# ritobanrc/firework

Measured on AMD Instinct MI355X. Metric: Mrays/s, cornell_box 512x512 @1024spp (scene resident in HBM; whole frame incl. tile gather), higher is better.
Workload: dtype f32; 1 GPU; C2_cornell_box 512x512 @1024spp; use_bvh=False, tiles=16x16, dealt diagonally over ranks, collective=none, rng=counter (pcg4d) keyed by (seed,pixel,sample,dimension), seed=0

## Files before the change

### firework_amd/csrc/fw_device.h

```cpp
#pragma once
#include <hip/hip_runtime.h>
#include <stdint.h>

#ifndef FW_AB
#define FW_AB 0
#endif

namespace fw {

constexpr int OBJ_Q = 6;

enum : uint32_t {
    OF_ROTATED = 1u << 0,
    OF_FLIP = 1u << 1,
    OF_RECT_FLIP = 1u << 2,
    OF_MESH_NORMALS = 1u << 3,
    OF_MESH_ATTR = 1u << 4,
    OF_CULL0 = 1u << 6,
    OF_GATE = 1u << 5,
};

constexpr uint32_t REF_LEAF = 0x80000000u, REF_DONE = 0xffffffffu;
constexpr int WIDE_NONE = 0, WIDE_F32 = 1, WIDE_Q8 = 2;
constexpr uint32_t WIDE_F32_DW = 28, WIDE_Q8_DW = 12;
// ... 226 lines not shown
    X(SHADE_GX_NEE_00_PL, "k_shade_gx_nee<0,0,pl>", -1) \
    X(SHADE_GX_NEE_01_PL, "k_shade_gx_nee<0,1,pl>", -1) \
    X(SHADE_GX_NEE_00_LS, "k_shade_gx_nee<0,0,ls>", -1) \
    X(SHADE_GX_NEE_01_LS, "k_shade_gx_nee<0,1,ls>", -1) \
    X(SHADE_GX_NEE_00_DL, "k_shade_gx_nee<0,0,dl>", -1) \
    X(SHADE_GX_NEE_01_DL, "k_shade_gx_nee<0,1,dl>", -1) \
    X(SHADE_GX_NEE_10_PL_ENV, "k_shade_gx_nee<1,0,pl_env>", -1) \
    X(SHADE_GX_NEE_10_ENV, "k_shade_gx_nee<1,0,env>", -1) \
    X(SHADE_GX_NEE_10_PL, "k_shade_gx_nee<1,0,pl>", -1) \
    X(SHADE_GX_NEE_11_PL, "k_shade_gx_nee<1,1,pl>", -1) \
    X(SHADE_GX_NEE_10_LS, "k_shade_gx_nee<1,0,ls>", -1) \
    X(SHADE_GX_NEE_11_LS, "k_shade_gx_nee<1,1,ls>", -1) \
    X(SHADE_GX_NEE_10_DL, "k_shade_gx_nee<1,0,dl>", -1) \
    X(SHADE_GX_NEE_11_DL, "k_shade_gx_nee<1,1,dl>", -1) \
    X(SHADE_GX_NEE_20_PL_ENV, "k_shade_gx_nee<2,0,pl_env>", -1) \
    X(SHADE_GX_NEE_20_ENV, "k_shade_gx_nee<2,0,env>", -1) \
    X(SHADE_GX_NEE_20_PL, "k_shade_gx_nee<2,0,pl>", -1) \
    X(SHADE_GX_NEE_21_PL, "k_shade_gx_nee<2,1,pl>", -1) \
    X(SHADE_GX_NEE_20_LS, "k_shade_gx_nee<2,0,ls>", -1) \
    X(SHADE_GX_NEE_21_LS, "k_shade_gx_nee<2,1,ls>", -1) \
    X(SHADE_GX_NEE_20_DL, "k_shade_gx_nee<2,0,dl>", -1) \
    X(SHADE_GX_NEE_21_DL, "k_shade_gx_nee<2,1,dl>", -1) \
    X(SHADOW_RESOLVE, "k_shadow_resolve", -1) \
    X(SHADOW_RESOLVE_ENV, "k_shadow_resolve_env", -1) \
    X(SHADOW_RESOLVE_PL, "k_shadow_resolve_pl", -1) \
    X(SHADOW_RESOLVE_DL, "k_shadow_resolve_dl", -1) \
    X(SHADOW_RESOLVE_GX, "k_shadow_resolve_gx", -1)
#if FW_AB
#define FW_KERNEL_IDS_AB(X) \
    X(EXTEND_BVH, "k_extend_bvh", -1) \
    X(SHADE_020, "k_shade<0,2,no chain>", -1) \
    X(SHADE_120, "k_shade<1,2,no chain>", -1) \
    X(SHADE_220, "k_shade<2,2,no chain>", -1) \
    X(BOUNCE_00, "k_bounce<false,false>", -1) \
    X(BOUNCE_01, "k_bounce<false,true>", -1) \
    X(BOUNCE_10, "k_bounce<true,false>", -1) \
    X(BOUNCE_11, "k_bounce<true,true>", -1)
#else
#define FW_KERNEL_IDS_AB(X)
#endif
#define FW_KERNEL_IDS(X) FW_KERNEL_IDS_PRODUCT(X) FW_KERNEL_IDS_AB(X)
enum KernelId : uint32_t {
#define FW_KID_ENUM(id, name, fam) KID_##id,
    FW_KERNEL_IDS(FW_KID_ENUM)
#undef FW_KID_ENUM
    KID_COUNT
};
constexpr uint32_t KID_N_WALK = 26;
extern const char *const KERNEL_NAMES[KID_COUNT];
extern const signed char KERNEL_FAMILY[KID_COUNT];
struct KernelLog {
    uint64_t bits[(KID_COUNT + 63) / 64];
    uint8_t waves[KID_COUNT];
    void clear() { *this = KernelLog{}; }
    void add(KernelId id) { bits[id >> 6] |= 1ull << (id & 63u); }
    void add(KernelId id, uint32_t w) { add(id); waves[id] |= (uint8_t)(w == 16u ? 1u : w == 12u ? 2u : 4u); }
    void merge(const KernelLog &o) { for (size_t i = 0; i < sizeof bits / sizeof bits[0]; i++) bits[i] |= o.bits[i]; for (uint32_t i = 0; i < KID_COUNT; i++) waves[i] |= o.waves[i]; }
    bool has(uint32_t id) const { return ((bits[id >> 6] >> (id & 63u)) & 1u) != 0; }
};

struct LaunchCfg {
    hipStream_t stream;
    DQueue q;
    int blocks_other;
    int tlas_depth, blas_depth;
    uint32_t n_mat, n_tex;
    bool lds_tables;
    bool has_mesh;
    bool simple_but_meshes;
    bool simple_set;
    int n_cus;
    uint32_t blas_pair_nodes, tlas_pair_nodes, max_tris, n_tris;
    bool no_lds_tris;
    uint32_t n_defer;
    bool lds_trees;
    int shade_mode;
    int exact_form;
    uint32_t ref_tlas_nodes, ref_blas_nodes, ref_tlas_depth, ref_blas_depth;
    int wblas_fmt, wtlas_fmt;
    uint32_t wblas_nodes, wtlas_nodes, wblas_depth, wtlas_depth;
    uint32_t debug_wide_levels;
    bool gx;
    KernelLog *log;
    bool tlas_refill;
};
constexpr size_t LDS_TREE_LIMIT = 160 * 1024;
constexpr size_t LDS_TABLE_LIMIT = 16 * 1024;

void launch_raygen(const LaunchCfg &, const DCamera &, const DFrame &, DPaths out, float4 *sample_rad, uint32_t n_paths);
void launch_raygen_views(const LaunchCfg &, const DCamera *cams, uint32_t n_view, const DFrame &, DPaths out, float4 *sample_rad, uint32_t n_paths);
void launch_resolve_views(const LaunchCfg &, const DFrame &, uint32_t n_view, const float4 *accum, uint32_t total_spp, float gamma,
                          uint8_t *rgb8, float *gamma_rgb, float *linear_rgb);
void launch_view_ids(hipStream_t stream, const uint32_t *src, uint32_t n_view, uint32_t n, uint32_t *out);
void launch_raygen_rays(const LaunchCfg &, const float *rays, bool per_sample, uint32_t *err, const DFrame &, DPaths out, uint32_t n_paths);
void launch_ray_keys(hipStream_t stream, uint32_t base, uint32_t n, uint32_t *out);
void launch_extend(const LaunchCfg &, const DScene &, const DFrame &, DPaths in, float2 *hits, int segment, bool use_bvh, DPark park);
void launch_extend_exact(const LaunchCfg &, const DScene &, const DFrame &, const DPaths &in, float2 *hits, int segment, bool use_bvh);
void launch_shade(const LaunchCfg &, const DScene &, const DFrame &, DPaths in, DPaths out, const float2 *hits,
                  float4 *sample_rad, int segment);
void launch_shade_nee(const LaunchCfg &, const DScene &, const DFrame &, DPaths in, DPaths out, const float2 *hits,
                      float4 *sample_rad, int segment, const DShadow &, const DEnvDist *ed, const DEmitters *em, const DDeltaLights *dl = nullptr);
void launch_shadow_resolve(const LaunchCfg &, const DScene &, const DShadow &, const float2 *hits, int segment, bool env, bool pl, bool dl = false,
                           float4 *sample_rad = nullptr);
int build_env_dist(hipStream_t stream, const DEnv &env, float *cdf_m, float *cdf_c, float *dens, float *p_out, double *scratch, double *total);
void launch_env_sample_test(hipStream_t stream, const DEnv &env, const DEnvDist &ed, uint32_t n, uint32_t seed32, float *out);
void launch_emitter_weights(hipStream_t stream, const DScene &sc, const uint4 *ent, uint32_t n, float *w);
void launch_emitter_sample_test(hipStream_t stream, const DScene &sc, const DEmitters &em, float x, float y, float z, uint32_t n, uint32_t seed32, float *out);
void launch_ggx_test(hipStream_t stream, uint32_t n, const float *in, float *out);
void launch_bounce(const LaunchCfg &, const DScene &, const DFrame &, DPaths in, DPaths out, float4 *sample_rad, int segment,
                   bool use_bvh);
void launch_queue_totals(const LaunchCfg &, uint32_t *totals, const uint32_t *ptotal);
void launch_trace_load(const LaunchCfg &, const DFrame &, const float *rays, DPaths out, uint32_t n, uint32_t key0, uint32_t *ids, uint32_t *slot_of);
void launch_trace_store(const LaunchCfg &, const DScene &, const DFrame &, const DPaths &in, const float2 *hits, const uint32_t *slot_of, uint32_t n,
                        float4 *out);
void launch_camera_rays(hipStream_t stream, int n_cus, const DCamera &, const DFrame &, uint32_t n, float *out);
void launch_aov_accumulate(hipStream_t stream, int n_cus, const DScene &, const DFrame &, const DPaths &in, const float2 *hits, const uint32_t *slot_of,
                           uint32_t n, uint32_t first, float4 *sum);
void launch_aov_finish(hipStream_t stream, int n_cus, uint32_t n, uint32_t spp, float4 *aov);
void launch_hit_surface(hipStream_t stream, int n_cus, const DScene &, uint32_t n_mat, const float *rays, const float4 *hits, uint32_t n, float4 *surface);
void launch_denoise(hipStream_t stream, int n_cus, uint32_t W, uint32_t H, uint32_t L, const float *color, const float4 *aov, const float4 *moments,
                    float4 *guide, float4 *ev0, float4 *ev1, float gamma, uint8_t *rgb8, float *gamma_rgb, float *linear_rgb);
void launch_scatter_tiles(hipStream_t stream, const uint32_t *ids, uint32_t n, const uint8_t *in8, const float *ing, const float *inl,
                          uint8_t *out8, float *outg, float *outl);
void launch_tile_order(hipStream_t stream, uint32_t width, uint32_t height, uint32_t *ids);
void launch_upload(hipStream_t stream, const void *pinned_src, void *dst, size_t bytes);
#if FW_AB
uint32_t take_error_word();
#endif
void preload_kernels();
void launch_count_deposits(const LaunchCfg &, const uint32_t *dep_bits, uint32_t *total);
void launch_selftest_arith(hipStream_t stream, uint32_t n, uint32_t seed, int mode, unsigned long long *out);
void launch_selftest_libm(hipStream_t stream, int fn, uint32_t n, const float *x, const float *y, float *out);
void launch_accumulate(const LaunchCfg &, const DFrame &, const float4 *sample_rad, float4 *accum);
void launch_resolve(const LaunchCfg &, const DFrame &, const float4 *accum, uint32_t total_spp, float gamma,
                    uint8_t *rgb8, float *gamma_rgb, float *linear_rgb);
constexpr uint32_t ADAPTIVE_MAX_BLOCKS = 1024;
void launch_accumulate_adaptive(const LaunchCfg &, const DFrame &, const float4 *sample_rad, float4 *accum, float4 *moments);
uint32_t adaptive_select_blocks(uint32_t n);
void launch_adaptive_select(hipStream_t stream, const uint32_t *ids, uint32_t n, const float4 *accum, float4 *moments, uint32_t n_samples, bool may_continue,
                            float tol, unsigned long long *mask, uint32_t *block_counts, uint32_t *out_ids, uint32_t *count);
void launch_resolve_adaptive(hipStream_t stream, int n_cus, uint32_t n, const float4 *accum, const float4 *moments, float gamma,
                             uint8_t *rgb8, float *gamma_rgb, float *linear_rgb);

constexpr int BLOCK = 256;

}
```

### firework_amd/csrc/fw_kernels.hip

```cpp
#include "../../include/firework_hip.h"
#include "fw_device.h"
#include "fw_libm.h"
#include "fw_defer_pretest.h"
#include <atomic>
#include <type_traits>

namespace fw {

struct V3 { float x, y, z; };
__device__ __forceinline__ V3 mk(float x, float y, float z) { return V3{x, y, z}; }
__device__ __forceinline__ V3 operator+(V3 a, V3 b) { return {a.x + b.x, a.y + b.y, a.z + b.z}; }
__device__ __forceinline__ V3 operator-(V3 a, V3 b) { return {a.x - b.x, a.y - b.y, a.z - b.z}; }
__device__ __forceinline__ V3 operator-(V3 a) { return {-a.x, -a.y, -a.z}; }
__device__ __forceinline__ V3 operator*(V3 a, V3 b) { return {a.x * b.x, a.y * b.y, a.z * b.z}; }
__device__ __forceinline__ V3 operator*(float s, V3 a) { return {s * a.x, s * a.y, s * a.z}; }
__device__ __forceinline__ V3 operator*(V3 a, float s) { return {a.x * s, a.y * s, a.z * s}; }
__device__ __forceinline__ float dot(V3 a, V3 b) { return fmaf(a.x, b.x, fmaf(a.y, b.y, a.z * b.z)); }
__device__ __forceinline__ V3 cross(V3 a, V3 b) {
    return {fmaf(a.y, b.z, -a.z * b.y), fmaf(a.z, b.x, -a.x * b.z), fmaf(a.x, b.y, -a.y * b.x)};
}
__device__ __forceinline__ float mag_sq(V3 a) { return dot(a, a); }
__device__ __forceinline__ float comp(V3 a, int i) { return i == 0 ? a.x : (i == 1 ? a.y : a.z); }
__device__ __forceinline__ V3 ld3(const float *p) { return {p[0], p[1], p[2]}; }

// ... 325 lines not shown
        const uint32_t slot = w * q.cap + chunk * 64u + lane;
        bool fl = false; V3 o = mk(0, 0, 0), d = o;
        if (i < n_paths) {
            const Ray r = camera_ray(cam, f, key_of_linear(f, i));
            o = r.o; d = r.d;
            if (f.pinhole0) qst(&out.ray_a[slot], make_float4(d.x, d.y, d.z, 0.f));
            else {
                qst(&out.ray_a[slot], make_float4(o.x, o.y, o.z, d.x));
                qst(&out.ray_b[slot], make_float2(d.y, d.z));
            }
            fl = f.ex.mode && needs_exact(f.ex, o.x, o.y, o.z, d.x, d.y, d.z);
        }
        if (f.ex.mode) flag_exact(f.ex, fl, slot, 0);
        produced += min(64u, n_paths - id0);
    }
    if (lane == 0) q.wcount[w] = produced;
}

__global__ __launch_bounds__(WB) void k_raygen_views(const DCamera *__restrict__ cams, uint32_t n_view, DFrame f, DPaths out,
                                                     float4 *__restrict__ sample_rad, DQueue q, uint32_t n_paths) {
    const uint32_t w = wave_index(), lane = threadIdx.x & 63u;
    if (w >= q.n_waves) return;
    uint32_t produced = 0;
    for (uint32_t chunk = 0;; chunk++) {
        uint32_t id0 = chunk * (q.n_waves * 64u) + w * 64u;
        if (id0 >= n_paths) break;
        uint32_t i = id0 + lane;
        const uint32_t slot = w * q.cap + chunk * 64u + lane;
        bool fl = false; V3 o = mk(0, 0, 0), d = o;
        if (i < n_paths) {
            uint32_t s_local = (uint32_t)((float)i * f.inv_n_pixels);
            int32_t p_local = (int32_t)(i - s_local * f.n_pixels);
            if (p_local < 0) p_local += (int32_t)f.n_pixels; else if ((uint32_t)p_local >= f.n_pixels) p_local -= (int32_t)f.n_pixels;
            const DCamera cam = cams[(uint32_t)p_local / n_view];
            const Ray r = camera_ray(cam, f, key_of_linear(f, i));
            o = r.o; d = r.d;
            if (f.pinhole0) qst(&out.ray_a[slot], make_float4(d.x, d.y, d.z, 0.f));
            else {
                qst(&out.ray_a[slot], make_float4(o.x, o.y, o.z, d.x));
                qst(&out.ray_b[slot], make_float2(d.y, d.z));
            }
            fl = f.ex.mode && needs_exact(f.ex, o.x, o.y, o.z, d.x, d.y, d.z);
        }
        if (f.ex.mode) flag_exact(f.ex, fl, slot, 0);
        produced += min(64u, n_paths - id0);
    }
    if (lane == 0) q.wcount[w] = produced;
}

struct Obj { float4 q0, q1, q2, q3, q4; uint32_t kf, material, aux0, aux1; };

__device__ __forceinline__ Obj load_obj(const float4 *__restrict__ objs, uint32_t j) {
    const float4 *p = objs + (size_t)j * OBJ_Q;
    float4 r0 = p[0], r3 = p[3], r4 = p[4], r5 = p[5];
    Obj o;
    o.q0 = make_float4(r3.x, r3.y, r3.z, r0.x); o.q1 = make_float4(r4.x, r4.y, r4.z, r0.y); o.q2 = make_float4(r5.x, r5.y, r5.z, r0.z);
    o.q3 = p[1]; o.q4 = p[2];
    o.kf = __float_as_uint(r0.w); o.material = __float_as_uint(r3.w);
    o.aux0 = __float_as_uint(r4.w); o.aux1 = __float_as_uint(r5.w);
    return o;
}
__device__ __forceinline__ Obj load_obj_for_hit(const float4 *__restrict__ objs, uint32_t j) {
    const float4 *p = objs + (size_t)j * OBJ_Q;
    float4 r0 = p[0];
    Obj o;
    o.kf = __float_as_uint(r0.w); o.material = 0; o.aux0 = 0; o.aux1 = 0;
    o.q0 = make_float4(1.f, 0.f, 0.f, r0.x); o.q1 = make_float4(0.f, 1.f, 0.f, r0.y); o.q2 = make_float4(0.f, 0.f, 1.f, r0.z);
    o.q3 = p[1]; o.q4 = make_float4(0.f, 0.f, 0.f, 0.f);
    const uint32_t kind = o.kf & 0xffu, flags = (o.kf >> 8) & 0xffffu, inner = o.kf >> 24;
    if (kind == 1u || kind == 2u || kind == 3u || kind == 4u || kind == 6u) o.q4 = p[2];
    const bool mesh = kind == 5u || (kind == 6u && inner == 5u);
    if ((flags & OF_ROTATED) || mesh) {
        float4 r3 = p[3], r4 = p[4], r5 = p[5];
        o.q0 = make_float4(r3.x, r3.y, r3.z, r0.x); o.q1 = make_float4(r4.x, r4.y, r4.z, r0.y); o.q2 = make_float4(r5.x, r5.y, r5.z, r0.z);
        o.aux0 = __float_as_uint(r4.w); o.aux1 = __float_as_uint(r5.w);
    }
    return o;
}
__device__ __forceinline__ uint32_t obj_kind(const Obj &o) { return o.kf & 0xffu; }
__device__ __forceinline__ uint32_t obj_flags(const Obj &o) { return (o.kf >> 8) & 0xffffu; }
__device__ __forceinline__ uint32_t obj_inner(const Obj &o) { return o.kf >> 24; }

__device__ __forceinline__ V3 rot_inv(const Obj &o, V3 v) {
    return {o.q0.x * v.x + o.q1.x * v.y + o.q2.x * v.z,
            o.q0.y * v.x + o.q1.y * v.y + o.q2.y * v.z,
            o.q0.z * v.x + o.q1.z * v.y + o.q2.z * v.z};
}
__device__ __forceinline__ V3 rot_fwd(const Obj &o, V3 v) {
    return {o.q0.x * v.x + o.q0.y * v.y + o.q0.z * v.z,
            o.q1.x * v.x + o.q1.y * v.y + o.q1.z * v.z,
            o.q2.x * v.x + o.q2.y * v.y + o.q2.z * v.z};
}
__device__ __forceinline__ Ray to_object_space(const Obj &o, const Ray &r) {
    V3 pos = mk(o.q0.w, o.q1.w, o.q2.w);
    if (obj_flags(o) & OF_ROTATED) return Ray{rot_inv(o, r.o - pos), rot_inv(o, r.d)};
    return Ray{r.o - pos, r.d};
}

__device__ __forceinline__ bool hit_sphere(float radius, const Ray &r, float tmin, float tmax, float &t_out) {
    float a = dot(r.d, r.d);
    float b = 2.f * dot(r.o, r.d);
    float c = dot(r.o, r.o) - radius * radius;
    float disc = b * b - 4.f * a * c;
    if (disc < 0.f) return false;
    float t1, t2; bool two;
    Rcp two_a = make_rcp(2.f * a);
// ... 867 lines not shown
        const float4 ra = ra_n; const float2 rb = rb_n;
        if (j + 64u < n) { ra_n = qld(&in.ray_a[i + 64u]); rb_n = load_ray_b(in, i + 64u, f, segment); }
        const bool active = j < n;
        bool deferred = false, have = false; uint32_t deferred_obj = 0, best_obj = MISS, best_prim = 0; float best_t = TMAX;
        Ray r{mk(0, 0, 0), mk(0, 0, 1)};
        if (active) {
            r = make_ray(ra, rb, f, segment);
            RngKey key{0, 0, 0};
            if (sc.has_medium) key = key_of(f, __float_as_uint(load_home(in, i, f, segment)));
            const V3 inv = mk(fdiv(1.f, r.d.x), fdiv(1.f, r.d.y), fdiv(1.f, r.d.z));
            const bool soft = sc.has_mesh && soft_ray(f.ex, r.d, sc.soft_shear);
            const uint32_t n_obj = skip_ray(f.ex, r) ? 0u : sc.n_objects;
            for (uint32_t k = 0; k < n_obj; k++) {
                const float4 lo = sc.obj_leaf[2 * (size_t)k], hi = sc.obj_leaf[2 * (size_t)k + 1];
                float entry;
                if (!hit_aabb_entry(lo, hi, r.o, inv, relaxed(inv), box_tmin(TMIN, soft), TMAX, entry) || entry > (soft ? NO_CULL : cull_bound(have ? best_t : TMAX))) continue;
                Obj o = load_obj(sc.obj, k);
                if (PARK && obj_kind(o) == 5u) {
                    if (obj_gate_ok(sc, k, r.o, inv)) { deferred = true; deferred_obj |= 1u << k; }
                    continue;
                }
                float t; uint32_t prim;
                if (PLAIN ? hit_object<false, 0, false, SIMPLE>(sc, o, k, r, TMIN, TMAX, nullptr, key, segment, t, prim) : hit_object(sc, o, k, r, TMIN, TMAX, blas_stack, key, segment, t, prim)) {
                    if ((!have || t < best_t || (t == best_t && sc.obj_rank[k] > sc.obj_rank[best_obj])) && obj_gate_ok(sc, k, r.o, inv)) { have = true; best_t = t; best_obj = k; best_prim = prim; }
                }
            }
            if (!deferred) qst(&hits[i], pack_hit(best_t, best_obj, best_prim, sc.prim_bits));
        }
        if (PARK) {
            const unsigned long long pmask = __ballot(deferred);
            if (pmask) {
                const uint32_t prank = __builtin_amdgcn_mbcnt_hi((uint32_t)(pmask >> 32), __builtin_amdgcn_mbcnt_lo((uint32_t)pmask, 0u));
                if (deferred) {
                    const uint32_t e = w * park_stride + park_n + prank;
                    qst(&park_a[e], make_float4(r.o.x, r.o.y, r.o.z, r.d.x));
                    qst(&park_b[e], make_float2(r.d.y, r.d.z));
                    qst(&park_m[e], make_float4(__uint_as_float(i), __uint_as_float(PARK_MASK | deferred_obj), best_t, pack_hit(best_t, best_obj, best_prim, sc.prim_bits).y));
                }
                park_n += (uint32_t)__popcll(pmask);
            }
        }
    }
    if (PARK && lane == 0) park_count[w] = park_n;
}

constexpr uint32_t DEFER_FIELDS = 9;
extern __shared__ uint32_t lds_defer[];
template <bool SIMPLE>
__global__ __launch_bounds__(WB) __attribute__((amdgpu_waves_per_eu(FW_DEFER_WAVES, 8)))
void k_extend_linear_defer(DScene sc, DFrame f, DPaths in, float2 *__restrict__ hits, DQueue q, int segment, uint32_t n_def) {
    const uint32_t w = wave_index(), lane = threadIdx.x & 63u;
    if (w >= q.n_waves) return;
    const uint32_t n = q.wcount[(size_t)segment * q.n_waves + w], base = w * q.cap;
    const float TMIN = 0.001f, TMAX = 2e9f;
    const uint32_t n_first = sc.n_objects - n_def;
    uint32_t *const L0 = lds_defer, *const L1 = lds_defer + DEFER_FIELDS * 64u;
    uint32_t cnt0 = 0, cnt1 = 0;
    const RngKey nokey{0, 0, 0};
    auto write_final = [&](uint32_t slot, float t, uint32_t code) {
        if (f.hit4) reinterpret_cast<uint32_t *>(hits)[slot] = code; else qst(&hits[slot], make_float2(t, __uint_as_float(code)));
    };
    auto put = [&](uint32_t *L, uint32_t e, uint32_t sb, float t, uint32_t code, const Ray &r) {
        L[e] = sb; L[64u + e] = __float_as_uint(t); L[128u + e] = code;
        L[192u + e] = __float_as_uint(r.o.x); L[256u + e] = __float_as_uint(r.o.y); L[320u + e] = __float_as_uint(r.o.z);
        L[384u + e] = __float_as_uint(r.d.x); L[448u + e] = __float_as_uint(r.d.y); L[512u + e] = __float_as_uint(r.d.z);
    };
    auto get = [&](const uint32_t *L, uint32_t e, uint32_t &sb, float &t, uint32_t &code, Ray &r) {
        sb = L[e]; t = __uint_as_float(L[64u + e]); code = L[128u + e];
        r.o = mk(__uint_as_float(L[192u + e]), __uint_as_float(L[256u + e]), __uint_as_float(L[320u + e]));
        r.d = mk(__uint_as_float(L[384u + e]), __uint_as_float(L[448u + e]), __uint_as_float(L[512u + e]));
    };
    auto test = [&](uint32_t d, const Ray &r, float &t, uint32_t &code) {
        const uint32_t k = n_first + d;
        const Obj o = load_obj(sc.obj, k);
        float tt; uint32_t prim;
        if (hit_rect3d(o.q3, o.q4, to_object_space(o, r), TMIN, t, tt, prim)) { t = tt; code = (k << sc.prim_bits) | prim; }
    };
    auto append = [&](uint32_t *L, uint32_t &cnt, bool want, uint32_t sb, float t, uint32_t code, const Ray &r) {
        const unsigned long long m = __ballot(want);
        if (!m) return;
        const uint32_t rank = __builtin_amdgcn_mbcnt_hi((uint32_t)(m >> 32), __builtin_amdgcn_mbcnt_lo((uint32_t)m, 0u));
        if (want) put(L, cnt + rank, sb, t, code, r);
        cnt += (uint32_t)__popcll(m);
    };
    auto make_room = [&](uint32_t need0, uint32_t need1) {
        const bool r0 = cnt0 != 0u && cnt0 + need0 > 64u;
        const uint32_t pass_on = r0 ? (uint32_t)__popcll(__ballot(lane < cnt0 && (L0[lane] >> 31) != 0u)) : 0u;
#pragma nounroll
        for (int phase = 0; phase < 2; phase++) {
            const bool r1 = cnt1 != 0u && (phase == 0 ? cnt1 + pass_on > 64u : cnt1 + need1 > 64u);
            if (r1) {
                uint32_t sb = 0, code = MISS; float t = TMAX; Ray r{mk(0, 0, 0), mk(0, 0, 1)};
                if (lane < cnt1) { get(L1, lane, sb, t, code, r); test(1, r, t, code); write_final(sb, t, code); }
                cnt1 = 0;
            }
            if (phase == 0 && r0) {
                uint32_t sb = 0, code = MISS; float t = TMAX; Ray r{mk(0, 0, 0), mk(0, 0, 1)};
                const bool on = lane < cnt0;
                if (on) { get(L0, lane, sb, t, code, r); test(0, r, t, code); }
                cnt0 = 0;
                const bool more = on && (sb >> 31) != 0u;
                const uint32_t slot = sb & 0x7fffffffu;
                if (on && !more) write_final(slot, t, code);
                append(L1, cnt1, more, slot, t, code, r);
            }
        }
    };
    float4 ra_n = make_float4(0, 0, 0, 0); float2 rb_n = make_float2(0, 0);
    if (lane < n) { ra_n = qld(&in.ray_a[base + lane]); rb_n = load_ray_b(in, base + lane, f, segment); }
    for (uint32_t c0 = 0; c0 < n; c0 += 64u) {
        const uint32_t j = c0 + lane, i = base + j;
        const float4 ra = ra_n; const float2 rb = rb_n;
        if (j + 64u < n) { ra_n = qld(&in.ray_a[i + 64u]); rb_n = load_ray_b(in, i + 64u, f, segment); }
        const bool active = j < n;
        float best_t = TMAX; uint32_t best_obj = MISS, best_prim = 0;
        bool may0 = false, may1 = false;
        const Ray r = make_ray(ra, rb, f, segment);
        if (active) {
            const float4 *op = sc.obj;
            const Rcp rcx = make_rcp(r.d.x), rcy = make_rcp(r.d.y), rcz = make_rcp(r.d.z);
            for (uint32_t k = 0; k < n_first; k++, op += OBJ_Q) {
                const Obj o = load_obj(op, 0);
                float t; uint32_t prim = 0; bool h;
                const uint32_t kind = obj_kind(o);
                if (kind >= 1u && kind <= 3u && !(obj_flags(o) & OF_ROTATED) && o.q4.y == 0.f) {
                    const Ray ro{r.o - mk(o.q0.w, o.q1.w, o.q2.w), r.d};
                    if (kind == 1u) h = hit_rect_rcp<0>(o.q3.x, o.q3.y, o.q3.z, o.q3.w, o.q4.x, ro, rcz, TMIN, best_t, t);
                    else if (kind == 2u) h = hit_rect_rcp<1>(o.q3.x, o.q3.y, o.q3.z, o.q3.w, o.q4.x, ro, rcy, TMIN, best_t, t);
                    else h = hit_rect_rcp<2>(o.q3.x, o.q3.y, o.q3.z, o.q3.w, o.q4.x, ro, rcx, TMIN, best_t, t);
                } else h = hit_object<false, 0, false, SIMPLE>(sc, o, k, r, TMIN, best_t, nullptr, nokey, segment, t, prim);
                if (h) { best_t = t; best_obj = k; best_prim = prim; }
            }
            const fwpt::RayTerms rt = fwpt::ray_terms(r.o.x, r.o.y, r.o.z, rcx.r, rcy.r, rcz.r);
            const float4 *const cb = sc.obj_cull + 2 * ((size_t)sc.n_objects + n_first);
            may0 = fwpt::pretest_fma(rt, cb[0].x, cb[0].y, cb[0].z, cb[1].x, cb[1].y, cb[1].z, best_t);
            if (n_def > 1u) may1 = fwpt::pretest_fma(rt, cb[2].x, cb[2].y, cb[2].z, cb[3].x, cb[3].y, cb[3].z, best_t);
        }
        const uint32_t code = best_obj == MISS ? MISS : ((best_obj << sc.prim_bits) | best_prim);
        const bool c1 = may1 && !may0;
        make_room((uint32_t)__popcll(__ballot(may0)), (uint32_t)__popcll(__ballot(c1)));
        if (active && !may0 && !may1) write_final(i, best_t, code);
        append(L0, cnt0, may0, i | (may1 ? 0x80000000u : 0u), best_t, code, r);
        append(L1, cnt1, c1, i, best_t, code, r);
    }
    make_room(65u, 65u);
}

__global__ __launch_bounds__(WB) __attribute__((amdgpu_waves_per_eu(7, 8)))
void k_extend_linear(DScene sc, DFrame f, DPaths in, float2 *__restrict__ hits, DQueue q, int segment, int tlas_levels, int stack_levels) {
    extend_body<false, false, false>(sc, f, in, hits, q, segment, tlas_levels, stack_levels, DPark{});
}
__global__ __launch_bounds__(WB) __attribute__((amdgpu_waves_per_eu(7, 8)))
void k_extend_linear_nomesh(DScene sc, DFrame f, DPaths in, float2 *__restrict__ hits, DQueue q, int segment, int tlas_levels, int stack_levels) {
    extend_body<false, false, false, false>(sc, f, in, hits, q, segment, tlas_levels, stack_levels, DPark{});
}
__global__ __launch_bounds__(WB) __attribute__((amdgpu_waves_per_eu(7, 8)))
void k_extend_linear_plain(DScene sc, DFrame f, DPaths in, float2 *__restrict__ hits, DQueue q, int segment, int tlas_levels, int stack_levels) {
    extend_body<false, false, false, false, false>(sc, f, in, hits, q, segment, tlas_levels, stack_levels, DPark{});
}
template <bool MEDIUM>
__global__ __launch_bounds__(WB) __attribute__((amdgpu_waves_per_eu(7, 8)))
void k_extend_linear_simple(DScene sc, DFrame f, DPaths in, float2 *__restrict__ hits, DQueue q, int segment, int tlas_levels, int stack_levels) {
    extend_body<false, false, false, false, MEDIUM, true>(sc, f, in, hits, q, segment, tlas_levels, stack_levels, DPark{});
}
#if FW_AB
__global__ __launch_bounds__(WB) __attribute__((amdgpu_waves_per_eu(5, 8)))
void k_extend_bvh(DScene sc, DFrame f, DPaths in, float2 *__restrict__ hits, DQueue q, int segment, int tlas_levels, int stack_levels) {
    extend_body<true, false, false>(sc, f, in, hits, q, segment, tlas_levels, stack_levels, DPark{});
}
#endif
__global__ __launch_bounds__(WB) __attribute__((amdgpu_waves_per_eu(FW_TLAS_WAVES, 8)))
void k_extend_tlas(DScene sc, DFrame f, DPaths in, float2 *__restrict__ hits, DQueue q, int segment, int tlas_levels, int stack_levels) {
    extend_body<true, true, false>(sc, f, in, hits, q, segment, tlas_levels, stack_levels, DPark{});
}
__global__ __launch_bounds__(WB) __attribute__((amdgpu_waves_per_eu(FW_TLAS_WAVES, 8)))
void k_extend_tlas_park(DScene sc, DFrame f, DPaths in, float2 *__restrict__ hits, DQueue q, int segment, int tlas_levels, int stack_levels, DPark park) {
    extend_body<true, true, true>(sc, f, in, hits, q, segment, tlas_levels, stack_levels, park);
}

__global__ __launch_bounds__(WB) __attribute__((amdgpu_waves_per_eu(FW_BLAS_WAVES, 8)))
void k_blas(DScene sc, DPark park, float2 *__restrict__ hits, DQueue q) {
    const uint32_t w = wave_index(), lane = threadIdx.x & 63u;
    if (w >= q.n_waves) return;
    TS_BEGIN();
    const uint32_t n = park.pcount[w];
    if (lane == 0 && n) park.ptotal[w] += n;
    const uint32_t base = w * park.stride;
    const float TMIN = 0.001f, TMAX = 2e9f;
    float4 ca = make_float4(0, 0, 0, 0), na = ca, cm = ca, nm = ca; float2 cb = make_float2(0, 0), nb = cb;
    auto fetch = [&](uint32_t j, float4 &a, float2 &b, float4 &m) {
        if (j < n) { a = qld(&park.ray_a[base + j]); b = qld(&park.ray_b[base + j]); m = qld(&park.meta[base + j]); }
    };
    fetch(lane, ca, cb, cm); fetch(64u + lane, na, nb, nm);
    uint32_t cur_base = 0, q_next = 0;
    bool act = false, have = false;
    uint32_t slot = 0, obj = 0, tri_base = 0, bcode = MISS, mtri = 0, cur = REF_DONE;
    float bt = TMAX, mbest = TMAX;
    V3 ro = mk(0, 0, 0), inv = ro;
// ... 1454 lines not shown
                    }
                }
            }
            if (CHAIN) nchain = chain | (o.material << (f.chain_bits * (uint32_t)segment));
            else {
                nbeta = beta * atten;
                if (f.atten && alive) f.atten[(size_t)segment * f.atten_stride + path_id] = make_float4(atten.x, atten.y, atten.z, 0.f);
            }
            PH_ADD(5);
        }
    }
#ifdef FW_ABL_NO_DEPOSIT
    if (false) {
#else
    if (!alive && !(f.skip_zero_deposits && rad.x == 0.f && rad.y == 0.f && rad.z == 0.f)) {
#endif
        PH_T0;
        const float len = (float)(segment + 1);
        if (LS) { const float4 e = sh->nee[path_id]; rad = rad + mk(e.x, e.y, e.z); }
        if (FW_NT_RAD) st_nt(&sample_rad[path_id], make_float4(rad.x, rad.y, rad.z, len));
        else sample_rad[path_id] = make_float4(rad.x, rad.y, rad.z, len);
        if (f.skip_zero_deposits) {
            const uint32_t b = f.dep_pixel_major ? dep_bit_of(f, path_id) : path_id;
            atomicOr(&f.dep_bits[b >> 5], 1u << (b & 31u));
        }
        PH_ADD(6);
    }
    return alive;
}

extern __shared__ float4 lds_tables[];

template <int LDS_TAB, int MODE, bool CHAIN>
#ifndef FW_SHADE_WAVES
#define FW_SHADE_WAVES 5
#endif
#ifndef FW_SHADE_PIPE
#define FW_SHADE_PIPE 0
#endif
#ifndef FW_SHADE_STATIC_STORES
#define FW_SHADE_STATIC_STORES FW_SHADE_PIPE
#endif
__attribute__((amdgpu_waves_per_eu(FW_SHADE_WAVES, 8)))
__global__ __launch_bounds__(WB) void k_shade(DScene sc, DFrame f, DPaths in, DPaths out, const float2 *__restrict__ hits,
                                                 float4 *__restrict__ sample_rad, DQueue q, int segment,
                                                 uint32_t n_mat, uint32_t n_tex) {
    const uint32_t w = wave_index(), lane = threadIdx.x & 63u;
    __shared__ uint16_t shade_list[128];
#include "fw_shade_tables.inc"
    if (w >= q.n_waves) return;
    const uint32_t n = q.wcount[(size_t)segment * q.n_waves + w];
    const uint32_t base = w * q.cap;
    uint32_t out_n = 0;
    uint32_t list_n = 0;
    PH_DECL;
    auto compact = [&](bool alive, const Ray &nr, V3 nbeta, uint32_t nchain, uint32_t path_id, uint32_t c0 = 0xffffffffu) {
        const unsigned long long mask = __ballot(alive);
        const uint32_t rank = __builtin_amdgcn_mbcnt_hi((uint32_t)(mask >> 32), __builtin_amdgcn_mbcnt_lo((uint32_t)mask, 0u));
#if FW_SHADE_STATIC_STORES
        if (c0 != 0xffffffffu) {
#if FW_SHADE_STATIC_STORES == 2
            const uint32_t dst = base + (alive ? out_n + rank : q.cap - 1u);
#else
            const uint32_t dst = base + (alive ? out_n + rank : min(c0 + 64u + lane, q.cap - 1u));
#endif
            qst(&out.ray_a[dst], make_float4(nr.o.x, nr.o.y, nr.o.z, nr.d.x));
            qst(&out.ray_b[dst], make_float2(nr.d.y, nr.d.z));
            if (CHAIN) qst(&reinterpret_cast<float2 *>(out.state)[dst], make_float2(__uint_as_float(nchain), __uint_as_float(path_id)));
            else qst(&out.state[dst], make_float4(nbeta.x, nbeta.y, nbeta.z, __uint_as_float(path_id)));
        } else
#endif
        if (alive) {
            const uint32_t dst = base + out_n + rank;
            qst(&out.ray_a[dst], make_float4(nr.o.x, nr.o.y, nr.o.z, nr.d.x));
            qst(&out.ray_b[dst], make_float2(nr.d.y, nr.d.z));
            if (CHAIN) qst(&reinterpret_cast<float2 *>(out.state)[dst], make_float2(__uint_as_float(nchain), __uint_as_float(path_id)));
            else qst(&out.state[dst], make_float4(nbeta.x, nbeta.y, nbeta.z, __uint_as_float(path_id)));
        }
        if (f.ex.mode)
            flag_exact(f.ex, alive && needs_exact(f.ex, nr.o.x, nr.o.y, nr.o.z, nr.d.x, nr.d.y, nr.d.z), base + out_n + rank, segment + 1);
        out_n += (uint32_t)__popcll(mask);
    };
    auto load_st = [&](uint32_t idx) { return CHAIN ? load_state_chain(in, idx, segment) : load_state(in, idx, segment); };
    auto load_hit = [&](uint32_t idx) { return f.hit4 ? make_float2(0.f, __uint_as_float(reinterpret_cast<const uint32_t *>(hits)[idx])) : qld(&hits[idx]); };
    auto run_list = [&](uint32_t take) {
        bool alive = false;
        Ray nr{mk(0, 0, 0), mk(0, 0, 0)}; V3 nbeta = mk(0, 0, 0); uint32_t path_id = 0, nchain = 0;
        if (lane < take) {
            const uint32_t i = base + shade_list[list_n - take + lane];
            const float4 ra = qld(&in.ray_a[i]), st = load_st(i); const float2 rb = load_ray_b(in, i, f, segment), hr = load_hit(i);
            path_id = __float_as_uint(st.w);
            alive = shade_path<false, CHAIN>(sc, f, objp, matp, texp, make_ray(ra, rb, f, segment), mk(st.x, st.y, st.z), __float_as_uint(st.x), path_id, hr.x, __float_as_uint(hr.y), segment, sample_rad, nr, nbeta, nchain PH_PASS);
        }
        list_n -= take;
        compact(alive, nr, nbeta, nchain, path_id);
    };
    float4 ra_n = make_float4(0, 0, 0, 0), st_n = ra_n; float2 rb_n = make_float2(0, 0), hr_n = rb_n;
#if FW_SHADE_PIPE
    auto prefetch = [&](uint32_t jn) {
        const uint32_t in_ = base + jn;
        ra_n = qld(&in.ray_a[in_]);
        rb_n = qld(&in.ray_b[short_rays(f, segment) ? base : in_]);
        if (CHAIN) { const float2 v = qld(&reinterpret_cast<const float2 *>(in.state)[segment == 0 ? base : in_]); st_n = make_float4(v.x, 0.f, 0.f, v.y); }
        else st_n = qld(&in.state[segment == 0 ? base : in_]);
        hr_n = load_hit(in_);
    };
    auto fix_implicit = [&](float4 &st_, float2 &rb_, uint32_t slot) {
        if (segment == 0) st_ = CHAIN ? make_float4(0.f, 0.f, 0.f, __uint_as_float(slot)) : make_float4(1.f, 1.f, 1.f, __uint_as_float(slot));
        if (short_rays(f, segment)) rb_ = make_float2(0.f, 0.f);
    };
    if (n) {
        prefetch(min(lane, n - 1u));
        const uint32_t d0 = base + lane;
        qst(&out.ray_a[d0], make_float4(0.f, 0.f, 0.f, 0.f));
        qst(&out.ray_b[d0], make_float2(0.f, 0.f));
        if (CHAIN) qst(&reinterpret_cast<float2 *>(out.state)[d0], make_float2(0.f, 0.f)); else qst(&out.state[d0], make_float4(0.f, 0.f, 0.f, 0.f));
    }
#else
    if (lane < n) { ra_n = qld(&in.ray_a[base + lane]); rb_n = load_ray_b(in, base + lane, f, segment); st_n = load_st(base + lane); hr_n = load_hit(base + lane); }
#endif
    for (uint32_t c0 = 0; c0 < n; c0 += 64u) {
        const uint32_t j = c0 + lane;
        const uint32_t i = base + j;
        float4 ra = ra_n, st = st_n; float2 rb = rb_n, hr = hr_n;
#if FW_SHADE_PIPE
        fix_implicit(st, rb, i);
        const RngKey key_ = key_of(f, __float_as_uint(st.w));
        prefetch(min(j + 64u, n - 1u));
        const RngKey *pre_key = &key_;
#else
        if (j + 64u < n) { ra_n = qld(&in.ray_a[i + 64u]); rb_n = load_ray_b(in, i + 64u, f, segment); st_n = load_st(i + 64u); hr_n = load_hit(i + 64u); }
        const RngKey *pre_key = nullptr;
#endif
        bool alive = false, later = false;
        Ray nr{mk(0, 0, 0), mk(0, 0, 0)}; V3 nbeta = mk(0, 0, 0); uint32_t path_id = 0, nchain = 0;
        if (j < n) {
            PH_T0;
            Ray r = make_ray(ra, rb, f, segment);
            V3 beta = mk(st.x, st.y, st.z);
            path_id = __float_as_uint(st.w);
            const uint32_t hit_code = __float_as_uint(hr.y);
#ifdef FW_ABL_SHADE_COPY
            alive = hit_code != MISS && segment < 10; nr = r; nbeta = beta; nchain = __float_as_uint(st.x) + (pre_key ? pre_key->pixel & 1u : 0u);
#else
            if (MODE == 2 && expensive_shading(sc, objp, matp, hit_code)) later = true;
            else alive = shade_path<MODE != 0, CHAIN>(sc, f, objp, matp, texp, r, beta, __float_as_uint(st.x), path_id, hr.x, hit_code, segment, sample_rad, nr, nbeta, nchain PH_PASS, pre_key);
#endif
            PH_ADD(0);
        }
        { PH_T0; compact(alive, nr, nbeta, nchain, path_id, c0); PH_ADD(7); }
        if (MODE == 2) {
            const unsigned long long lm = __ballot(later);
            if (lm) {
                const uint32_t lr = __builtin_amdgcn_mbcnt_hi((uint32_t)(lm >> 32), __builtin_amdgcn_mbcnt_lo((uint32_t)lm, 0u));
                if (later) shade_list[list_n + lr] = (uint16_t)j;
                list_n += (uint32_t)__popcll(lm);
                if (list_n >= 64u) run_list(64u);
            }
        }
    }
    if (MODE == 2) while (list_n) run_list(min(list_n, 64u));
    if (lane == 0) q.wcount[(size_t)(segment + 1) * q.n_waves + w] = out_n;
    PH_FLUSH(1);
}
template <int LDS_TAB, int MODE>
__attribute__((amdgpu_waves_per_eu(FW_SHADE_WAVES, 8)))
__global__ __launch_bounds__(WB) void k_shade_ls(DScene sc, DFrame f, DPaths in, DPaths out, const float2 *__restrict__ hits,
                                                    float4 *__restrict__ sample_rad, DQueue q, int segment,
                                                    uint32_t n_mat, uint32_t n_tex, DShadow sh) {
    constexpr bool ENV = false, PL = false, DL = false, GX = false;
    const DEnvDist *const edp = nullptr; const DEmitters *const emp = nullptr; const DDeltaLights *const dlp = nullptr;
#include "fw_shade_nee.inc"
}
template <int LDS_TAB>
__attribute__((amdgpu_waves_per_eu(FW_SHADE_WAVES, 8)))
__global__ __launch_bounds__(WB) void k_shade_env(DScene sc, DFrame f, DPaths in, DPaths out, const float2 *__restrict__ hits,
                                                     float4 *__restrict__ sample_rad, DQueue q, int segment,
                                                     uint32_t n_mat, uint32_t n_tex, DShadow sh, DEnvDist ed) {
    constexpr int MODE = 0;
    constexpr bool ENV = true, PL = false, DL = false, GX = false;
    const DEnvDist *const edp = &ed; const DEmitters *const emp = nullptr; const DDeltaLights *const dlp = nullptr;
#include "fw_shade_nee.inc"
}
__global__ __launch_bounds__(WB) void k_shadow_resolve(DShadow sh, const float2 *__restrict__ hits, DQueue q, int segment, uint32_t prim_bits) {
    const uint32_t w = wave_index(), lane = threadIdx.x & 63u;
    if (w >= q.n_waves) return;
    const uint32_t n = sh.wcount[(size_t)(segment + 1) * q.n_waves + w], base = w * q.cap;
    for (uint32_t j = lane; j < n; j += 64u) {
        const uint32_t i = base + j, code = __float_as_uint(hits[i].y);
        if (code == MISS || (code >> prim_bits) != sh.obj[i]) continue;
        const float4 p = sh.state[i];
        float4 &e = sh.nee[__float_as_uint(p.w)];
        e = make_float4(e.x + p.x, e.y + p.y, e.z + p.z, 0.f);
    }
}
__global__ __launch_bounds__(WB) void k_shadow_resolve_env(DShadow sh, const float2 *__restrict__ hits, DQueue q, int segment, uint32_t prim_bits) {
    const uint32_t w = wave_index(), lane = threadIdx.x & 63u;
    if (w >= q.n_waves) return;
    const uint32_t n = sh.wcount[(size_t)(segment + 1) * q.n_waves + w], base = w * q.cap;
    for (uint32_t j = lane; j < n; j += 64u) {
        const uint32_t i = base + j, code = __float_as_uint(hits[i].y);
        if ((code == MISS ? MISS : code >> prim_bits) != sh.obj[i]) continue;
        const float4 p = sh.state[i];
        float4 &e = sh.nee[__float_as_uint(p.w)];
        e = make_float4(e.x + p.x, e.y + p.y, e.z + p.z, 0.f);
    }
}
template <int LDS_TAB, int MODE>
__attribute__((amdgpu_waves_per_eu(FW_SHADE_WAVES, 8)))
__global__ __launch_bounds__(WB) void k_shade_pl(DScene sc, DFrame f, DPaths in, DPaths out, const float2 *__restrict__ hits,
                                                    float4 *__restrict__ sample_rad, DQueue q, int segment,
                                                    uint32_t n_mat, uint32_t n_tex, DShadow sh, DEmitters em) {
    constexpr bool ENV = false, PL = true, DL = false, GX = false;
    const DEnvDist *const edp = nullptr; const DEmitters *const emp = &em; const DDeltaLights *const dlp = nullptr;
#include "fw_shade_nee.inc"
}
// ... 670 lines not shown
__global__ __launch_bounds__(BLOCK) void k_ray_keys(uint32_t base, uint32_t n, uint32_t *__restrict__ out) {
    for (uint32_t i = blockIdx.x * BLOCK + threadIdx.x; i < n; i += gridDim.x * BLOCK) out[i] = base + i;
}

static dim3 wave_grid(const LaunchCfg &c) { return dim3((c.q.n_waves + WB / 64 - 1) / (WB / 64)); }
void launch_trace_load(const LaunchCfg &c, const DFrame &f, const float *rays, DPaths out, uint32_t n, uint32_t key0, uint32_t *ids, uint32_t *slot_of) {
    hipLaunchKernelGGL(k_trace_load, wave_grid(c), dim3(WB), 0, c.stream, f, rays, out, c.q, n, key0, ids, slot_of);
}
void launch_trace_store(const LaunchCfg &c, const DScene &sc, const DFrame &f, const DPaths &in, const float2 *hits, const uint32_t *slot_of, uint32_t n,
                        float4 *out) {
    const uint32_t blocks = (uint32_t)std::max<uint64_t>(1, std::min<uint64_t>(((uint64_t)n + BLOCK - 1) / BLOCK, (uint64_t)c.n_cus * 32u));
    hipLaunchKernelGGL(k_trace_store, dim3(blocks), dim3(BLOCK), 0, c.stream, sc, f, in, hits, slot_of, n, out);
}
void launch_camera_rays(hipStream_t stream, int n_cus, const DCamera &cam, const DFrame &f, uint32_t n, float *out) {
    const uint32_t blocks = (uint32_t)std::max<uint64_t>(1, std::min<uint64_t>(((uint64_t)n + 63u) / 64u, (uint64_t)n_cus * 64u));
    hipLaunchKernelGGL(k_camera_rays, dim3(blocks), dim3(WB), 0, stream, cam, f, n, out);
}

void launch_raygen(const LaunchCfg &c, const DCamera &cam, const DFrame &f, DPaths out, float4 *sample_rad, uint32_t n_paths) {
    hipLaunchKernelGGL(k_raygen, wave_grid(c), dim3(WB), 0, c.stream, cam, f, out, sample_rad, c.q, n_paths);
}
void launch_raygen_views(const LaunchCfg &c, const DCamera *cams, uint32_t n_view, const DFrame &f, DPaths out, float4 *sample_rad, uint32_t n_paths) {
    hipLaunchKernelGGL(k_raygen_views, wave_grid(c), dim3(WB), 0, c.stream, cams, n_view, f, out, sample_rad, c.q, n_paths);
}
void launch_raygen_rays(const LaunchCfg &c, const float *rays, bool per_sample, uint32_t *err, const DFrame &f, DPaths out, uint32_t n_paths) {
    hipLaunchKernelGGL(k_raygen_rays, wave_grid(c), dim3(WB), 0, c.stream, rays, per_sample ? 1u : 0u, err, f, out, c.q, n_paths);
}
void launch_ray_keys(hipStream_t stream, uint32_t base, uint32_t n, uint32_t *out) {
    hipLaunchKernelGGL(k_ray_keys, dim3(std::min<uint32_t>((n + BLOCK - 1) / BLOCK, 4096u)), dim3(BLOCK), 0, stream, base, n, out);
}
void launch_resolve_views(const LaunchCfg &c, const DFrame &f, uint32_t n_view, const float4 *accum, uint32_t total_spp, float gamma,
                          uint8_t *rgb8, float *gamma_rgb, float *linear_rgb) {
    hipLaunchKernelGGL(k_resolve_views, dim3(c.blocks_other), dim3(BLOCK), 0, c.stream, f, n_view, accum, total_spp, gamma, rgb8, gamma_rgb, linear_rgb);
}
void launch_view_ids(hipStream_t stream, const uint32_t *src, uint32_t n_view, uint32_t n, uint32_t *out) {
    hipLaunchKernelGGL(k_view_ids, dim3(std::min<uint32_t>((n + BLOCK - 1) / BLOCK, 4096u)), dim3(BLOCK), 0, stream, src, n_view, n, out);
}
static bool lds_attr_needed(int which) {
    static std::atomic<unsigned char> done[4][64];
    int dev = 0;
    if (hipGetDevice(&dev) != hipSuccess || dev < 0 || dev >= 64) return true;
    return done[which][dev].exchange(1) == 0;
}
static size_t lds_walk_bytes(size_t tree_bytes, uint32_t waves, uint32_t levels, uint32_t n_queues, uint32_t grid) {
    return tree_bytes + (size_t)waves * levels * 64 * 2 + 16 + 4 * (size_t)((n_queues + grid - 1) / grid);
}
#define FW_LAUNCH(ID, ...) do { if (c.log) c.log->add(KID_##ID); hipLaunchKernelGGL(__VA_ARGS__); } while (0)
#define FW_LAUNCH_W(ID, W, ...) do { if (c.log) c.log->add(KID_##ID, (uint32_t)(W)); hipLaunchKernelGGL(__VA_ARGS__); } while (0)
const char *const KERNEL_NAMES[KID_COUNT] = {
#define FW_KID_NAME(id, name, fam) name,
    FW_KERNEL_IDS(FW_KID_NAME)
#undef FW_KID_NAME
};
const signed char KERNEL_FAMILY[KID_COUNT] = {
#define FW_KID_FAM(id, name, fam) fam,
    FW_KERNEL_IDS(FW_KID_FAM)
#undef FW_KID_FAM
};
void launch_extend(const LaunchCfg &c, const DScene &sc, const DFrame &f, DPaths in, float2 *hits, int segment, bool use_bvh, DPark park) {
    int tl = use_bvh ? c.tlas_depth + 1 : 0;
    int levels = tl + c.blas_depth + 1;
    size_t lds = (size_t)levels * WB * sizeof(uint32_t) + (use_bvh && c.has_mesh ? 5 * DEFER_CAP * sizeof(uint32_t) : 0);
    dim3 eg = wave_grid(c);
    const dim3 sg = eg;
    auto walk_grid = [&](uint32_t waves) { return std::min<uint32_t>((uint32_t)c.n_cus, (c.q.n_waves + waves - 1) / waves); };
    if (use_bvh && c.tlas_refill && c.has_mesh) {
        if (sc.n_objects <= TLAS_SCAN_MAX && !sc.has_medium && c.simple_but_meshes) FW_LAUNCH(EXTEND_SCAN_PARK_NM_S, (k_extend_scan<true, true, true>), eg, dim3(WB), (size_t)levels * WB * sizeof(uint32_t), c.stream, sc, f, in, hits, c.q, segment, tl, park.ray_a, park.ray_b, park.meta, park.pcount, park.stride);
        else if (sc.n_objects <= TLAS_SCAN_MAX && !sc.has_medium) FW_LAUNCH(EXTEND_SCAN_PARK_NM, (k_extend_scan<true, true>), eg, dim3(WB), (size_t)levels * WB * sizeof(uint32_t), c.stream, sc, f, in, hits, c.q, segment, tl, park.ray_a, park.ray_b, park.meta, park.pcount, park.stride);
        else if (sc.n_objects <= TLAS_SCAN_MAX) FW_LAUNCH(EXTEND_SCAN_PARK, k_extend_scan<true>, eg, dim3(WB), (size_t)levels * WB * sizeof(uint32_t), c.stream, sc, f, in, hits, c.q, segment, tl, park.ray_a, park.ray_b, park.meta, park.pcount, park.stride);
        else FW_LAUNCH(EXTEND_TLAS_PARK, k_extend_tlas_park, sg, dim3(WB), (size_t)levels * WB * sizeof(uint32_t), c.stream, sc, f, in, hits, c.q, segment, tl, levels, park);
        if (c.lds_trees && c.wblas_fmt != WIDE_NONE && sc.wblas && c.max_tris < 0x7fffu) {
            const uint32_t wl = c.debug_wide_levels ? c.debug_wide_levels : 3u * c.wblas_depth + 2u;
            const size_t tree = (size_t)c.wblas_nodes * (c.wblas_fmt == WIDE_F32 ? WIDE_F32_DW : WIDE_Q8_DW) * 4, tris = (size_t)c.n_tris * 48;
            uint32_t waves = 0; bool lds_tris = false;
            if (!c.no_lds_tris && lds_walk_bytes(tree + tris, 16, wl, c.q.n_waves, walk_grid(16)) <= LDS_TREE_LIMIT) { waves = 16; lds_tris = true; }
            else for (uint32_t w : {16u, 12u, 8u}) if (lds_walk_bytes(tree, w, wl, c.q.n_waves, walk_grid(w)) <= LDS_TREE_LIMIT) { waves = w; break; }
            if (waves) {
                if (lds_attr_needed(2)) {
                    (void)hipFuncSetAttribute(reinterpret_cast<const void *>(k_blas_wide<WIDE_F32, false>), hipFuncAttributeMaxDynamicSharedMemorySize, (int)LDS_TREE_LIMIT);
                    (void)hipFuncSetAttribute(reinterpret_cast<const void *>(k_blas_wide<WIDE_F32, true>), hipFuncAttributeMaxDynamicSharedMemorySize, (int)LDS_TREE_LIMIT);
                    (void)hipFuncSetAttribute(reinterpret_cast<const void *>(k_blas_wide<WIDE_Q8, false>), hipFuncAttributeMaxDynamicSharedMemorySize, (int)LDS_TREE_LIMIT);
                    (void)hipFuncSetAttribute(reinterpret_cast<const void *>(k_blas_wide<WIDE_Q8, true>), hipFuncAttributeMaxDynamicSharedMemorySize, (int)LDS_TREE_LIMIT);
                }
                const dim3 lg(walk_grid(waves));
                const size_t bytes = lds_walk_bytes(tree + (lds_tris ? tris : 0), waves, wl, c.q.n_waves, lg.x);
#define FW_BLAS_WIDE(ID, F, T) FW_LAUNCH_W(ID, waves, (k_blas_wide<F, T>), lg, dim3(waves * 64), bytes, c.stream, sc, park, hits, c.q, c.wblas_nodes, c.n_tris, wl)
                if (c.wblas_fmt == WIDE_F32) { if (lds_tris) FW_BLAS_WIDE(BLAS_WIDE_F32_T, WIDE_F32, true); else FW_BLAS_WIDE(BLAS_WIDE_F32_N, WIDE_F32, false); }
                else { if (lds_tris) FW_BLAS_WIDE(BLAS_WIDE_Q8_T, WIDE_Q8, true); else FW_BLAS_WIDE(BLAS_WIDE_Q8_N, WIDE_Q8, false); }
#undef FW_BLAS_WIDE
                return;
            }
        }
        const uint32_t bl = (uint32_t)c.blas_depth + 1u;
        const size_t lds_blas = lds_walk_bytes((size_t)c.blas_pair_nodes * 64, LDS_WAVES, bl, c.q.n_waves, walk_grid(LDS_WAVES)), lds_tris = (size_t)c.n_tris * 48;
        if (c.lds_trees && c.blas_pair_nodes > 0 && c.blas_pair_nodes < 32768u && c.max_tris < 32768u && lds_blas <= LDS_TREE_LIMIT) {
            if (lds_attr_needed(0)) {
                (void)hipFuncSetAttribute(reinterpret_cast<const void *>(k_blas_lds<false>), hipFuncAttributeMaxDynamicSharedMemorySize, (int)LDS_TREE_LIMIT);
                (void)hipFuncSetAttribute(reinterpret_cast<const void *>(k_blas_lds<true>), hipFuncAttributeMaxDynamicSharedMemorySize, (int)LDS_TREE_LIMIT);
            }
            const dim3 lg(walk_grid(LDS_WAVES));
            if (lds_blas + lds_tris <= LDS_TREE_LIMIT && !c.no_lds_tris)
                FW_LAUNCH_W(BLAS_LDS_T, LDS_WAVES, k_blas_lds<true>, lg, dim3(LDS_WAVES * 64), lds_blas + lds_tris, c.stream, sc, park, hits, c.q, c.blas_pair_nodes, c.n_tris, bl);
            else
                FW_LAUNCH_W(BLAS_LDS_N, LDS_WAVES, k_blas_lds<false>, lg, dim3(LDS_WAVES * 64), lds_blas, c.stream, sc, park, hits, c.q, c.blas_pair_nodes, c.n_tris, bl);
        }
        else FW_LAUNCH(BLAS, k_blas, sg, dim3(WB), (size_t)(c.blas_depth + 1) * WB * sizeof(uint32_t), c.stream, sc, park, hits, c.q);
// ... 23 lines not shown
        if (c.lds_trees && !c.has_mesh && sc.n_objects > TLAS_SCAN_MAX && c.tlas_pair_nodes < 32768u && sc.n_objects < 32768u && lds_tlas <= LDS_TREE_LIMIT) {
            if (lds_attr_needed(1)) (void)hipFuncSetAttribute(reinterpret_cast<const void *>(k_extend_tlas_lds), hipFuncAttributeMaxDynamicSharedMemorySize, (int)LDS_TREE_LIMIT);
            FW_LAUNCH_W(EXTEND_TLAS_LDS, LDS_WAVES, k_extend_tlas_lds, dim3(walk_grid(LDS_WAVES)), dim3(LDS_WAVES * 64), lds_tlas, c.stream,
                               sc, f, in, hits, c.q, segment, c.tlas_pair_nodes, (uint32_t)tl);
        }
        else if (sc.n_objects <= TLAS_SCAN_MAX) FW_LAUNCH(EXTEND_SCAN, k_extend_scan<false>, eg, dim3(WB), lds, c.stream, sc, f, in, hits, c.q, segment, tl, (float4 *)nullptr, (float2 *)nullptr, (float4 *)nullptr, (uint32_t *)nullptr, 0u);
        else FW_LAUNCH(EXTEND_TLAS, k_extend_tlas, sg, dim3(WB), lds, c.stream, sc, f, in, hits, c.q, segment, tl, levels);
    }
#if FW_AB
    else if (use_bvh) FW_LAUNCH(EXTEND_BVH, k_extend_bvh, eg, dim3(WB), lds, c.stream, sc, f, in, hits, c.q, segment, tl, levels);
#endif
    else if (c.n_defer && c.simple_set) FW_LAUNCH(EXTEND_LINEAR_DEFER_S, k_extend_linear_defer<true>, eg, dim3(WB), (size_t)2 * 64 * DEFER_FIELDS * 4 + FW_DEFER_LDS_PAD, c.stream, sc, f, in, hits, c.q, segment, c.n_defer);
    else if (c.n_defer) FW_LAUNCH(EXTEND_LINEAR_DEFER_N, k_extend_linear_defer<false>, eg, dim3(WB), (size_t)2 * 64 * DEFER_FIELDS * 4 + FW_DEFER_LDS_PAD, c.stream, sc, f, in, hits, c.q, segment, c.n_defer);
    else if (c.simple_set && !sc.has_medium) FW_LAUNCH(EXTEND_LINEAR_SIMPLE_N, k_extend_linear_simple<false>, eg, dim3(WB), lds, c.stream, sc, f, in, hits, c.q, segment, tl, levels);
    else if (c.simple_set) FW_LAUNCH(EXTEND_LINEAR_SIMPLE_M, k_extend_linear_simple<true>, eg, dim3(WB), lds, c.stream, sc, f, in, hits, c.q, segment, tl, levels);
    else if (!c.has_mesh && !sc.has_medium) FW_LAUNCH(EXTEND_LINEAR_PLAIN, k_extend_linear_plain, eg, dim3(WB), lds, c.stream, sc, f, in, hits, c.q, segment, tl, levels);
    else if (!c.has_mesh) FW_LAUNCH(EXTEND_LINEAR_NOMESH, k_extend_linear_nomesh, eg, dim3(WB), lds, c.stream, sc, f, in, hits, c.q, segment, tl, levels);
    else FW_LAUNCH(EXTEND_LINEAR, k_extend_linear, eg, dim3(WB), lds, c.stream, sc, f, in, hits, c.q, segment, tl, levels);
}
void launch_extend_exact(const LaunchCfg &c, const DScene &sc, const DFrame &f, const DPaths &in, float2 *hits, int segment, bool use_bvh) {
    const uint32_t tl = std::max<uint32_t>(std::min<uint32_t>(c.ref_tlas_depth + 2u, EXACT_LEVELS), (EXACT_STACK + 2u * EXACT_DEFER) / EXACT_WB);
    const uint32_t bl = std::max<uint32_t>(std::min<uint32_t>(c.ref_blas_depth + 2u, EXACT_LEVELS), EXACT_STACK / EXACT_WB);
    const size_t lds = (size_t)(tl + bl) * EXACT_WB * 4;
    FW_LAUNCH(EXTEND_EXACT, k_extend_exact, dim3((uint32_t)c.n_cus * 8u), dim3(EXACT_WB), lds, c.stream, sc, f, in, hits, segment, use_bvh ? 1 : 0, tl, c.exact_form);
}
struct ShadeTables { int lt; size_t lds; };
static void launch_shade_gx(const LaunchCfg &c, const DScene &sc, const DFrame &f, DPaths in, DPaths out, const float2 *hits, float4 *sample_rad, int segment, const ShadeTables &t);
static void launch_shade_gx_nee(const LaunchCfg &c, const DScene &sc, const DFrame &f, DPaths in, DPaths out, const float2 *hits, float4 *sample_rad, int segment,
                                const DShadow &sh, const DEnvDist *ed, const DEmitters *em, const DDeltaLights *dl, const ShadeTables &t);
static void launch_shadow_resolve_gx(const LaunchCfg &c, const DScene &sc, const DShadow &sh, const float2 *hits, int segment, float4 *sample_rad);
static ShadeTables shade_tables(const LaunchCfg &c, const DScene &sc) {
    const size_t tab_mt = (2 * (size_t)c.n_mat + 2 * (size_t)c.n_tex) * sizeof(float4), tab = (size_t)sc.n_objects * OBJ_Q * sizeof(float4) + tab_mt;
    if (c.lds_tables && tab <= LDS_TABLE_LIMIT) return {1, tab};
    if (c.lds_tables && tab_mt <= LDS_TABLE_LIMIT) return {2, tab_mt};
    return {0, 0};
}
void launch_shade(const LaunchCfg &c, const DScene &sc, const DFrame &f, DPaths in, DPaths out, const float2 *hits,
                  float4 *sample_rad, int segment) {
    const ShadeTables t = shade_tables(c, sc);
    if (c.gx) { launch_shade_gx(c, sc, f, in, out, hits, sample_rad, segment, t); return; }
    const int mode = c.shade_mode;
#define FW_SHADE(L, M, C, CI) FW_LAUNCH(SHADE_##L##M##CI, (k_shade<L, M, C>), wave_grid(c), dim3(WB), t.lds, c.stream, sc, f, in, out, hits, sample_rad, c.q, segment, c.n_mat, c.n_tex)
#define FW_SHADE_C(L, M) do { if (f.chain_bits) FW_SHADE(L, M, true, 1); else FW_SHADE(L, M, false, 0); } while (0)
#if FW_AB
#define FW_SHADE_L(L) do { if (mode == 2) FW_SHADE(L, 2, false, 0); else if (mode == 1) FW_SHADE_C(L, 1); else FW_SHADE_C(L, 0); } while (0)
#else
#define FW_SHADE_L(L) do { if (mode == 1) FW_SHADE_C(L, 1); else FW_SHADE_C(L, 0); } while (0)
#endif
    if (t.lt == 1) FW_SHADE_L(1); else if (t.lt == 2) FW_SHADE_L(2); else FW_SHADE_L(0);
#undef FW_SHADE_L
#undef FW_SHADE_C
#undef FW_SHADE
}
void launch_shade_nee(const LaunchCfg &c, const DScene &sc, const DFrame &f, DPaths in, DPaths out, const float2 *hits,
                      float4 *sample_rad, int segment, const DShadow &sh, const DEnvDist *ed, const DEmitters *em, const DDeltaLights *dl) {
    const ShadeTables t = shade_tables(c, sc);
    const bool m1 = c.shade_mode == 1;
    if (c.gx) { launch_shade_gx_nee(c, sc, f, in, out, hits, sample_rad, segment, sh, ed, em, dl, t); return; }
#define FW_NEE(ID, K, ...) FW_LAUNCH(ID, K, wave_grid(c), dim3(WB), t.lds, c.stream, sc, f, in, out, hits, sample_rad, c.q, segment, c.n_mat, c.n_tex, __VA_ARGS__)
#define FW_NEE_L(L) do { \
        if (ed && em) FW_NEE(SHADE_PL_ENV_##L, k_shade_pl_env<L>, sh, *ed, *em); \
        else if (ed) FW_NEE(SHADE_ENV_##L, k_shade_env<L>, sh, *ed); \
        else if (em) { if (m1) FW_NEE(SHADE_PL_##L##1, (k_shade_pl<L, 1>), sh, *em); else FW_NEE(SHADE_PL_##L##0, (k_shade_pl<L, 0>), sh, *em); } \
        else if (!dl) { if (m1) FW_NEE(SHADE_LS_##L##1, (k_shade_ls<L, 1>), sh); else FW_NEE(SHADE_LS_##L##0, (k_shade_ls<L, 0>), sh); } \
        else { if (m1) FW_NEE(SHADE_DL_##L##1, (k_shade_dl<L, 1>), sh, *dl); else FW_NEE(SHADE_DL_##L##0, (k_shade_dl<L, 0>), sh, *dl); } \
    } while (0)
    if (t.lt == 1) FW_NEE_L(1); else if (t.lt == 2) FW_NEE_L(2); else FW_NEE_L(0);
#undef FW_NEE_L
#undef FW_NEE
}
void launch_shadow_resolve(const LaunchCfg &c, const DScene &sc, const DShadow &sh, const float2 *hits, int segment, bool env, bool pl, bool dl, float4 *sample_rad) {
    if (c.gx && !env && !pl) { launch_shadow_resolve_gx(c, sc, sh, hits, segment, sample_rad); return; }
    if (dl) FW_LAUNCH(SHADOW_RESOLVE_DL, k_shadow_resolve_dl, wave_grid(c), dim3(WB), 0, c.stream, sh, hits, c.q, segment, sc.prim_bits);
    else if (pl) FW_LAUNCH(SHADOW_RESOLVE_PL, k_shadow_resolve_pl, wave_grid(c), dim3(WB), 0, c.stream, sh, hits, c.q, segment);
    else if (env) FW_LAUNCH(SHADOW_RESOLVE_ENV, k_shadow_resolve_env, wave_grid(c), dim3(WB), 0, c.stream, sh, hits, c.q, segment, sc.prim_bits);
    else FW_LAUNCH(SHADOW_RESOLVE, k_shadow_resolve, wave_grid(c), dim3(WB), 0, c.stream, sh, hits, c.q, segment, sc.prim_bits);
}
void launch_emitter_weights(hipStream_t stream, const DScene &sc, const uint4 *ent, uint32_t n, float *w) {
    hipLaunchKernelGGL(k_emitter_weights, dim3((n + WB - 1) / WB), dim3(WB), 0, stream, sc, ent, n, w);
}
void launch_emitter_sample_test(hipStream_t stream, const DScene &sc, const DEmitters &em, float x, float y, float z, uint32_t n, uint32_t seed32, float *out) {
    hipLaunchKernelGGL(k_emitter_sample_test, dim3((n + WB - 1) / WB), dim3(WB), 0, stream, sc, em, x, y, z, n, seed32, out);
}
int build_env_dist(hipStream_t stream, const DEnv &env, float *cdf_m, float *cdf_c, float *dens, float *p_out, double *scratch, double *total) {
    const size_t n = (size_t)env.hdr_w * env.hdr_h;
    hipLaunchKernelGGL(k_env_rows, dim3(env.hdr_h), dim3(ENV_BUILD_THREADS), 0, stream, env, cdf_c, scratch);
    hipLaunchKernelGGL(k_env_marg, dim3(1), dim3(ENV_BUILD_THREADS), 0, stream, env.hdr_h, cdf_m, scratch);
    hipLaunchKernelGGL(k_env_dens, dim3((unsigned)((n + ENV_BUILD_THREADS - 1) / ENV_BUILD_THREADS)), dim3(ENV_BUILD_THREADS), 0, stream, env, dens, p_out,
                       (const double *)scratch);
    if (hipGetLastError() != hipSuccess) return FW_ERR_HIP;
    if (hipMemcpyAsync(total, scratch + env.hdr_h, sizeof(double), hipMemcpyDeviceToHost, stream) != hipSuccess) return FW_ERR_HIP;
    if (hipStreamSynchronize(stream) != hipSuccess) return FW_ERR_HIP;
    return FW_OK;
}
void launch_env_sample_test(hipStream_t stream, const DEnv &env, const DEnvDist &ed, uint32_t n, uint32_t seed32, float *out) {
    hipLaunchKernelGGL(k_env_sample_test, dim3((n + WB - 1) / WB), dim3(WB), 0, stream, env, ed, n, seed32, out);
}
#if FW_AB
void launch_bounce(const LaunchCfg &c, const DScene &sc, const DFrame &f, DPaths in, DPaths out, float4 *sample_rad,
                   int segment, bool use_bvh) {
    const ShadeTables t = shade_tables(c, sc);
    const bool lds_tab = t.lt == 1;
    const size_t tab = lds_tab ? t.lds : 0;
    int tl = use_bvh ? c.tlas_depth + 1 : 0;
    int levels = tl + c.blas_depth + 1;
    size_t lds = tab + (size_t)levels * WB * sizeof(uint32_t);
    uint32_t tq = (uint32_t)(tab / sizeof(float4));
    dim3 g = wave_grid(c);
#define FW_BOUNCE(ID, B, T) FW_LAUNCH(ID, (k_bounce<B, T>), g, dim3(WB), lds, c.stream, sc, f, in, out, sample_rad, c.q, segment, tl, c.n_mat, c.n_tex, tq)
    if (use_bvh) { if (lds_tab) FW_BOUNCE(BOUNCE_11, true, true); else FW_BOUNCE(BOUNCE_10, true, false); }
    else { if (lds_tab) FW_BOUNCE(BOUNCE_01, false, true); else FW_BOUNCE(BOUNCE_00, false, false); }
#undef FW_BOUNCE
}
#endif
void preload_kernels() {
    hipFuncAttributes a;
#define FW_TOUCH(k) (void)hipFuncGetAttributes(&a, reinterpret_cast<const void *>(k))
    FW_TOUCH(k_raygen); FW_TOUCH(k_extend_linear); FW_TOUCH(k_extend_linear_nomesh); FW_TOUCH(k_extend_linear_plain); FW_TOUCH(k_extend_linear_defer<true>); FW_TOUCH(k_extend_linear_defer<false>); FW_TOUCH(k_extend_linear_simple<true>); FW_TOUCH(k_extend_linear_simple<false>); FW_TOUCH(k_extend_scan<true>); FW_TOUCH((k_extend_scan<true, true>)); FW_TOUCH((k_extend_scan<true, true, true>)); FW_TOUCH(k_extend_scan<false>);
    FW_TOUCH(k_extend_tlas); FW_TOUCH(k_extend_tlas_park); FW_TOUCH(k_blas); FW_TOUCH(k_blas_lds<true>); FW_TOUCH(k_blas_lds<false>); FW_TOUCH(k_extend_tlas_lds);
    FW_TOUCH((k_blas_wide<WIDE_F32, true>)); FW_TOUCH((k_blas_wide<WIDE_F32, false>)); FW_TOUCH((k_blas_wide<WIDE_Q8, true>)); FW_TOUCH((k_blas_wide<WIDE_Q8, false>));
    FW_TOUCH(k_extend_tlas_wide<true>); FW_TOUCH(k_extend_tlas_wide<false>); FW_TOUCH((k_extend_tlas_wide<true, true>)); FW_TOUCH((k_extend_tlas_wide<false, true>)); FW_TOUCH(k_extend_exact); FW_TOUCH(k_queue_totals); FW_TOUCH(k_count_deposits); FW_TOUCH(k_accumulate); FW_TOUCH(k_tile_order);
    FW_TOUCH(k_resolve); FW_TOUCH(k_raygen_views); FW_TOUCH(k_resolve_views); FW_TOUCH(k_view_ids); FW_TOUCH(k_raygen_rays); FW_TOUCH(k_ray_keys); FW_TOUCH(k_accumulate_adaptive); FW_TOUCH(k_adaptive_select); FW_TOUCH(k_adaptive_compact); FW_TOUCH(k_resolve_adaptive); FW_TOUCH(k_scatter_tiles); FW_TOUCH(k_trace_load); FW_TOUCH(k_trace_store); FW_TOUCH(k_camera_rays);
    FW_TOUCH((k_shade<0, 0, false>)); FW_TOUCH((k_shade<0, 0, true>)); FW_TOUCH((k_shade<0, 1, false>)); FW_TOUCH((k_shade<0, 1, true>));
    FW_TOUCH((k_shade<1, 0, false>)); FW_TOUCH((k_shade<1, 0, true>)); FW_TOUCH((k_shade<1, 1, false>)); FW_TOUCH((k_shade<1, 1, true>));
    FW_TOUCH((k_shade<2, 0, false>)); FW_TOUCH((k_shade<2, 0, true>)); FW_TOUCH((k_shade<2, 1, false>)); FW_TOUCH((k_shade<2, 1, true>));
#undef FW_TOUCH
    (void)hipGetLastError();
}
#if FW_AB
uint32_t take_error_word() {
    uint32_t v = 0, zero = 0;
    if (hipMemcpyFromSymbol(&v, HIP_SYMBOL(g_err_word), 4) != hipSuccess) { (void)hipGetLastError(); return 0; }
    if (v) (void)hipMemcpyToSymbol(HIP_SYMBOL(g_err_word), &zero, 4);
    return v;
}
#endif
#ifdef FW_PHASE_STATS
extern "C" int fw_debug_phase_stats(unsigned long long *out, int n) {
    static unsigned long long zero[2 * 3 * PH_N];
    if (n < 2 * 3 * PH_N) return -1;
    if (hipMemcpyFromSymbol(out, HIP_SYMBOL(g_phase), sizeof zero) != hipSuccess) return -1;
    return hipMemcpyToSymbol(HIP_SYMBOL(g_phase), zero, sizeof zero) == hipSuccess ? 2 * 3 * PH_N : -1;
}
#endif
#ifdef FW_TRAV_STATS
extern "C" int fw_debug_trav_stats(unsigned long long out[8]) {
    unsigned long long zero[8] = {0, 0, 0, 0, 0, 0, 0, 0};
    if (hipMemcpyFromSymbol(out, HIP_SYMBOL(g_trav), sizeof zero) != hipSuccess) return -1;
    return hipMemcpyToSymbol(HIP_SYMBOL(g_trav), zero, sizeof zero) == hipSuccess ? 0 : -1;
}
#endif
void launch_queue_totals(const LaunchCfg &c, uint32_t *totals, const uint32_t *ptotal) {
    hipLaunchKernelGGL(k_queue_totals, dim3(32, MAX_SEGMENTS + 1), dim3(BLOCK), 0, c.stream, c.q, totals, ptotal);
}
void launch_count_deposits(const LaunchCfg &c, const uint32_t *dep_bits, uint32_t *total) {
    hipLaunchKernelGGL(k_count_deposits, dim3(1024), dim3(BLOCK), 0, c.stream, dep_bits, (c.q.n_waves * c.q.cap + 31u) / 32u, total);
}
void launch_accumulate(const LaunchCfg &c, const DFrame &f, const float4 *sample_rad, float4 *accum) {
    uint32_t blocks = (uint32_t)std::max<uint64_t>(1, std::min<uint64_t>(((uint64_t)f.n_pixels + WB - 1) / WB, 65536));
    hipLaunchKernelGGL(k_accumulate, dim3(blocks), dim3(WB), 0, c.stream, f, sample_rad, accum);
}
void launch_resolve(const LaunchCfg &c, const DFrame &f, const float4 *accum, uint32_t total_spp, float gamma,
                    uint8_t *rgb8, float *gamma_rgb, float *linear_rgb) {
    hipLaunchKernelGGL(k_resolve, dim3(c.blocks_other), dim3(BLOCK), 0, c.stream, f, accum, total_spp, gamma, rgb8, gamma_rgb, linear_rgb);
}
void launch_accumulate_adaptive(const LaunchCfg &c, const DFrame &f, const float4 *sample_rad, float4 *accum, float4 *moments) {
    uint32_t blocks = (uint32_t)std::max<uint64_t>(1, std::min<uint64_t>(((uint64_t)f.n_pixels + WB - 1) / WB, 65536));
    hipLaunchKernelGGL(k_accumulate_adaptive, dim3(blocks), dim3(WB), 0, c.stream, f, sample_rad, accum, moments);
}
void launch_resolve_adaptive(hipStream_t stream, int n_cus, uint32_t n, const float4 *accum, const float4 *moments, float gamma,
                             uint8_t *rgb8, float *gamma_rgb, float *linear_rgb) {
    const uint32_t blocks = (uint32_t)std::max<uint64_t>(1, std::min<uint64_t>(((uint64_t)n + BLOCK - 1) / BLOCK, (uint64_t)n_cus * 8));
    hipLaunchKernelGGL(k_resolve_adaptive, dim3(blocks), dim3(BLOCK), 0, stream, n, accum, moments, gamma, rgb8, gamma_rgb, linear_rgb);
}
uint32_t adaptive_select_blocks(uint32_t n) { return (uint32_t)std::max<uint64_t>(1, std::min<uint64_t>(((uint64_t)n + BLOCK - 1) / BLOCK, ADAPTIVE_MAX_BLOCKS)); }
void launch_adaptive_select(hipStream_t stream, const uint32_t *ids, uint32_t n, const float4 *accum, float4 *moments, uint32_t n_samples, bool may_continue,
                            float tol, unsigned long long *mask, uint32_t *block_counts, uint32_t *out_ids, uint32_t *count) {
    const uint32_t blocks = adaptive_select_blocks(n), per_block = (n + blocks - 1) / blocks, per = (per_block + BLOCK - 1) / BLOCK * BLOCK;
// ... 297 lines not shown
```

### firework_amd/csrc/fw_runtime.cpp

```cpp
#include "../../include/firework_hip.h"
#include "fw_device.h"
#include "fw_build.h"
#include "fw_temporal.h"
#include "fw_camera_models.h"
#include "fw_probes.h"
#include "fw_lightmap.h"
#include "fw_probe_lookup.h"
#include "fw_probe_depth.h"
#include "fw_ao.h"
#include "fw_probe_place.h"
#include "fw_probe_radiance.h"
#include "fw_direct.h"
#include "fw_sky.h"
#include "fw_ggx_table.h"
#include "fw_gather.h"
#include "fw_reflect.h"
#include "fw_area.h"
#include "fw_defer_pretest.h"

#include <algorithm>
#include <atomic>
#include <exception>
#include <chrono>
#include <cmath>
#include <cstdio>
#include <cstdlib>
#include <cstring>
#include <limits>
#include <mutex>
#include <new>
#include <string>
#include <thread>
#include <vector>

namespace {

thread_local std::string g_last_error;

int fail(int status, const std::string &msg) { g_last_error = msg; return status; }

struct Options {
    bool bvh_median = false;
    bool no_exact = false, exact_all = false;
    int exact_form = 0;
    bool no_defer = false, no_hit4 = false, no_hoist = false, no_lds_tables = false, no_lds_trees = false, no_lds_tris = false, no_short_rays = false,
         no_tile_order = false, no_zero_skip = false, dep_pixel_major = false, dep_slot_major = false, trace = false, no_chain = false,
         exact_product = false;
    int streams = 0;
    int graph = -1;
    int phase_lock = -1;
    int soft_shear_log2 = 5, exact_shear_log2 = 10; double exact_far_x = 256.0;
    double wide_node_cost = 0.0005;
    int wide = -1;
    int build = -1;
    long waves = 0;
    long long paths_per_batch = 0;
    std::string dump_path;
#if FW_AB
    bool fused = false, tlas_refill_off = false, shade_list = false, no_shade_defer = false, stagger = false;
    int debug_wide_levels = 0;
#endif
};
const char *const OPTION_NAMES[] = {"BVH", "NO_EXACT", "EXACT_ALL", "EXACT_FORM", "NO_DEFER", "NO_HIT4", "NO_HOIST", "NO_LDS_TABLES", "NO_LDS_TREES", "NO_LDS_TRIS",
                                    "NO_SHORT_RAYS", "NO_TILE_ORDER", "NO_ZERO_SKIP", "DEP_PIXEL_MAJOR", "DEP_SLOT_MAJOR", "NO_CHAIN", "EXACT_PRODUCT", "PHASE_LOCK", "GRAPH", "SOFT_SHEAR_LOG2", "EXACT_SHEAR_LOG2", "EXACT_FAR_X", "WIDE_NODE_COST", "TRACE", "STREAMS", "WIDE", "BUILD", "WAVES",
                                    "PATHS_PER_BATCH", "DUMP_PATH",
#if FW_AB
                                    "FUSED", "TLAS_REFILL", "SHADE_LIST", "NO_SHADE_DEFER", "STAGGER", "DEBUG_WIDE_LEVELS",
#endif
                                    nullptr};
bool option_apply(Options &o, const char *name, const char *v) {
    const std::string n = name;
    auto on = [&] { return v != nullptr; };
    auto num = [&] { return v ? atoll(v) : 0ll; };
    if (n == "BVH") o.bvh_median = v && std::strcmp(v, "median") == 0;
    else if (n == "NO_EXACT") o.no_exact = on();
    else if (n == "EXACT_ALL") o.exact_all = num() != 0;
    else if (n == "EXACT_FORM") o.exact_form = v ? (std::strcmp(v, "lane") == 0 ? 1 : (std::strcmp(v, "wave") == 0 ? 2 : 0)) : 0;
    else if (n == "NO_DEFER") o.no_defer = on();
    else if (n == "NO_HIT4") o.no_hit4 = on();
    else if (n == "NO_HOIST") o.no_hoist = on();
    else if (n == "NO_LDS_TABLES") o.no_lds_tables = on();
    else if (n == "NO_LDS_TREES") o.no_lds_trees = on();
    else if (n == "NO_LDS_TRIS") o.no_lds_tris = on();
    else if (n == "NO_SHORT_RAYS") o.no_short_rays = on();
    else if (n == "NO_TILE_ORDER") o.no_tile_order = on();
    else if (n == "NO_ZERO_SKIP") o.no_zero_skip = on();
    else if (n == "DEP_PIXEL_MAJOR") o.dep_pixel_major = on();
    else if (n == "DEP_SLOT_MAJOR") o.dep_slot_major = on();
    else if (n == "NO_CHAIN") o.no_chain = on();
    else if (n == "EXACT_PRODUCT") o.exact_product = v && atoi(v) != 0;
    else if (n == "PHASE_LOCK") o.phase_lock = v ? (atoi(v) != 0 ? 1 : 0) : -1;
    else if (n == "GRAPH") o.graph = v ? (atoi(v) != 0 ? 1 : 0) : -1;
    else if (n == "SOFT_SHEAR_LOG2") o.soft_shear_log2 = v ? (int)num() : 5;
    else if (n == "EXACT_SHEAR_LOG2") o.exact_shear_log2 = v ? (int)num() : 10;
    else if (n == "EXACT_FAR_X") o.exact_far_x = v ? atof(v) : 256.0;
    else if (n == "WIDE_NODE_COST") o.wide_node_cost = v ? atof(v) : 0.0005;
    else if (n == "TRACE") o.trace = on();
    else if (n == "STREAMS") o.streams = (int)std::max<long long>(0, num());
    else if (n == "WIDE") o.wide = !v ? -1 : (std::strcmp(v, "0") == 0 ? 0 : (std::strcmp(v, "f32") == 0 ? 1 : (std::strcmp(v, "q8") == 0 ? 2 : -1)));
    else if (n == "BUILD") {
        if (v && std::strcmp(v, "host") != 0 && std::strcmp(v, "device") != 0) return false;
        o.build = !v ? -1 : (std::strcmp(v, "device") == 0 ? 1 : 0);
    }
    else if (n == "WAVES") o.waves = (long)std::max<long long>(0, num());
    else if (n == "PATHS_PER_BATCH") o.paths_per_batch = std::max<long long>(0, num());
    else if (n == "DUMP_PATH") o.dump_path = v ? v : "";
#if FW_AB
    else if (n == "FUSED") o.fused = num() != 0;
    else if (n == "TLAS_REFILL") o.tlas_refill_off = v && atoi(v) == 0;
    else if (n == "SHADE_LIST") o.shade_list = on();
    else if (n == "NO_SHADE_DEFER") o.no_shade_defer = on();
    else if (n == "STAGGER") o.stagger = on();
    else if (n == "DEBUG_WIDE_LEVELS") o.debug_wide_levels = (int)std::max<long long>(0, num());
#endif
    else return false;
    return true;
}
Options options_from_env() {
    Options o;
    for (int k = 0; OPTION_NAMES[k]; k++) { const std::string e = std::string("FIREWORK_") + OPTION_NAMES[k]; if (const char *v = getenv(e.c_str())) option_apply(o, OPTION_NAMES[k], v); }
    return o;
}
std::mutex g_opt_mu;
Options g_opt = options_from_env();
Options options() { std::lock_guard<std::mutex> g(g_opt_mu); return g_opt; }

#define HIPCHK(expr)                                                                                           \
    do {                                                                                                       \
        hipError_t e_ = (expr);                                                                                \
        if (e_ != hipSuccess) {                                                                                \
            char buf_[512];                                                                                    \
            snprintf(buf_, sizeof buf_, "%s failed: %s (%s:%d)", #expr, hipGetErrorString(e_), __FILE__, __LINE__); \
            return fail(e_ == hipErrorOutOfMemory ? FW_ERR_OOM : FW_ERR_HIP, buf_);                            \
        }                                                                                                      \
    } while (0)

int need_device(int *n_out = nullptr) {
    int ndev = 0;
    if (hipGetDeviceCount(&ndev) != hipSuccess || ndev <= 0) { (void)hipGetLastError(); return fail(FW_ERR_NO_DEVICE, "no HIP device visible (this library has no CPU path)"); }
    if (n_out) *n_out = ndev;
    return FW_OK;
}
int use_device(int device) {
    int ndev = 0;
// ... 1742 lines not shown
    if (n == 0) { sc->n_dlights = 0; return FW_OK; }
    if (sc->d.n_objects >= fw::SHADOW_NEAR) return fail(FW_ERR_UNSUPPORTED, "too many objects for a scene with lights");
    const std::vector<float> rec = light_records(lights, n);
    const size_t bytes = rec.size() * 4, total = (bytes + 255) & ~(size_t)255;
    HIPCHK(hipSetDevice(sc->device));
    Workspace *ws = workspace_for(sc->device);
    if (!ws) return fail(FW_ERR_OOM, "no workspace for this device");
    std::lock_guard<std::mutex> ws_guard(ws->mu);
    if (int rc = init_device_locked(ws, sc->device)) return rc;
    if (int rc = staging_reserve_locked(ws, total)) return rc;
    if (sc->dlights.bytes < total || !sc->dlights.p) {
        DevBuf nb;
        if (int rc = nb.alloc(total)) return rc;
        sc->dlights.release();
        sc->dlights = nb;
    }
    uint8_t *blob = (uint8_t *)ws->staging;
    std::memset(blob, 0, total);
    std::memcpy(blob, rec.data(), bytes);
    sc->n_dlights = 0;
    fw::launch_upload(ws->upload_stream, blob, sc->dlights.p, total);
    if (hipEventRecord(ws->ev_upload, ws->upload_stream) != hipSuccess || hipGetLastError() != hipSuccess) return fail(FW_ERR_HIP, "light upload failed");
    sc->n_dlights = n;
    return FW_OK;
}

fw::DCamera make_camera(const fw_camera_settings &s, uint32_t width, uint32_t height) {
    const float PI_F = 3.14159265358979323846f;
    float theta = s.vfov * PI_F / 180.f;
    V3 cam_pos = tov(s.cam_pos), look_at = tov(s.look_at);
    V3 w = normalized(cam_pos - look_at);
    V3 u = normalized(cross(V3{0, 1, 0}, w));
    V3 v = cross(w, u);
    float half_height = std::tan(theta / 2.0f);
    float half_width = half_height * (float)width / (float)height;
    V3 lower_left = cam_pos - half_width * s.focus_dist * u - half_height * s.focus_dist * v - w * s.focus_dist;
    V3 horizontal = 2.0f * half_width * s.focus_dist * u;
    V3 vertical = 2.0f * half_height * s.focus_dist * v;
    fw::DCamera c;
    auto put = [](float *d, V3 a) { d[0] = a.x; d[1] = a.y; d[2] = a.z; };
    put(c.position, cam_pos); put(c.horizontal, horizontal); put(c.vertical, vertical); put(c.lower_left, lower_left); put(c.u, u); put(c.v, v);
    c.lens_radius = s.aperture / 2.f;
    return c;
}

uint32_t default_paths_per_batch(const Options &O, size_t arena_bytes) {
    if (O.paths_per_batch > 0) return (uint32_t)std::min<long long>(O.paths_per_batch, 0x7fffffffll);
    size_t free_b = 0, total_b = 0;
    uint64_t budget = 1ull << 28;
    if (hipMemGetInfo(&free_b, &total_b) == hipSuccess && free_b + arena_bytes > 0) budget = std::min<uint64_t>(budget, (uint64_t)((free_b + arena_bytes) / 2) / 288u);
    return (uint32_t)std::max<uint64_t>(budget, 1u << 16);
}

void set_walk_cfg(fw::LaunchCfg &cfg, const fw_scene *sc, const Options &O, const fw::DQueue &q, bool use_bvh, bool tlas_refill) {
    cfg.q = q;
    cfg.tlas_depth = (int)sc->tlas_depth; cfg.blas_depth = (int)sc->blas_depth;
    cfg.n_mat = sc->n_mat; cfg.n_tex = sc->n_tex;
    cfg.lds_tables = !O.no_lds_tables;
    cfg.has_mesh = sc->d.has_mesh != 0;
    cfg.simple_set = sc->simple_set; cfg.simple_but_meshes = sc->simple_but_meshes;
#ifdef FW_NO_SIMPLE
    cfg.simple_set = cfg.simple_but_meshes = false;
#endif
    cfg.tlas_refill = tlas_refill;
    cfg.n_cus = sc->n_cus;
    cfg.blas_pair_nodes = sc->blas_pair_nodes; cfg.tlas_pair_nodes = sc->tlas_pair_nodes; cfg.max_tris = sc->max_tris; cfg.n_tris = sc->n_tris;
    cfg.no_lds_tris = O.no_lds_tris;
    cfg.n_defer = (!use_bvh && !O.no_defer) ? sc->n_defer : 0u;
    cfg.lds_trees = !O.no_lds_trees;
    cfg.wblas_fmt = sc->wblas_fmt; cfg.wtlas_fmt = sc->wtlas_fmt; cfg.wblas_nodes = sc->wblas_nodes; cfg.wtlas_nodes = sc->wtlas_nodes;
    cfg.wblas_depth = sc->wblas_depth; cfg.wtlas_depth = sc->wtlas_depth;
    cfg.exact_form = O.exact_form;
    cfg.debug_wide_levels = 0;
#if FW_AB
    cfg.debug_wide_levels = (uint32_t)O.debug_wide_levels;
#endif
    cfg.ref_tlas_nodes = sc->tlas_nodes; cfg.ref_blas_nodes = sc->blas_nodes; cfg.ref_tlas_depth = sc->ref_tlas_depth; cfg.ref_blas_depth = sc->ref_blas_depth;
}

static bool light_sampling(const fw_scene *sc, const fw_render_params *p) {
    return (p->flags & FW_FLAG_LIGHT_SAMPLING) != 0 && sc->n_lights > 0 && sc->ls_vertices;
}
static bool delta_lights(const fw_scene *sc) { return sc->n_dlights > 0 && sc->ls_vertices; }
static int build_env_table(const fw::DEnv &env, DevBuf &buf, float *p_out, double &total, hipEvent_t after = nullptr) {
    const size_t n = (size_t)env.hdr_w * env.hdr_h;
    if (int rc = buf.alloc((env.hdr_h + 2 * n) * 4)) return rc;
    DevBuf scratch;
    if (int rc = scratch.alloc((2 * (size_t)env.hdr_h + 1) * 8)) return rc;
    float *base = (float *)buf.p;
    if (after && hipStreamWaitEvent(nullptr, after, 0) != hipSuccess) { scratch.release(); return fail(FW_ERR_HIP, "hipStreamWaitEvent failed"); }
    const int rc = fw::build_env_dist(nullptr, env, base, base + env.hdr_h, base + env.hdr_h + n, p_out, (double *)scratch.p, &total);
    scratch.release();
    return rc ? fail(rc, "environment table build failed") : FW_OK;
}
static fw::DEnvDist env_dist_of(const DevBuf &buf, const fw::DEnv &env, float p_env) {
    const float *base = (const float *)buf.p;
    const size_t n = (size_t)env.hdr_w * env.hdr_h;
    return fw::DEnvDist{base, base + env.hdr_h, base + env.hdr_h + n, p_env, env.hdr_w, env.hdr_h};
}
static int ensure_env_dist(fw_scene *sc, const fw_render_params *p, const Workspace *ws) {
    if (!(p->flags & FW_FLAG_ENV_SAMPLING) || sc->d.env.kind != FW_ENV_HDR || !sc->ls_vertices || sc->env_state != 0) return FW_OK;
    if ((uint64_t)sc->d.env.hdr_w * sc->d.env.hdr_h > 0xffffffffull) { sc->env_state = 2; return FW_OK; }
    const auto t0 = std::chrono::steady_clock::now();
    double total = 0;
    if (int rc = build_env_table(sc->d.env, sc->env_dist, nullptr, total, ws->ev_upload)) return rc;
    sc->env_state = total > 0 ? 1 : 2;
// ... 112 lines not shown

struct RayInput { const float *rays; uint32_t n; bool per_sample; const uint32_t *keys; uint32_t key_base; bool on_device; };

int render_impl(fw_scene *sc, const fw_render_params *p, uint8_t *rgb8, float *gamma_rgb, float *linear_rgb, fw_stats *stats,
                uint32_t first_sample = 0, float *user_accum = nullptr, const AdaptiveRound *rd = nullptr, const ViewGroup *vg = nullptr,
                const RayInput *ri = nullptr) {
    if (!sc || !p) return fail(FW_ERR_BAD_ARG, "null argument");
    if (p->width == 0 || p->height == 0 || p->samples == 0) return fail(FW_ERR_BAD_ARG, "width, height and samples must be > 0");
    if (!(p->gamma > 0.f)) return fail(FW_ERR_BAD_ARG, "gamma must be > 0");
    if (p->rng_mode != FW_RNG_CTR) return fail(FW_ERR_UNSUPPORTED, "the HIP path implements FW_RNG_CTR only (FW_RNG_LCG is a sequential stream)");
    uint64_t full = (uint64_t)p->width * p->height;
    if (full > 0xffffffffull) return fail(FW_ERR_UNSUPPORTED, "image too large");
    const uint32_t n_view = rd ? rd->n : ri ? ri->n : (p->pixel_ids ? p->n_pixels : (uint32_t)full);
    if (n_view == 0) return fail(FW_ERR_BAD_ARG, "no pixels to render");
    if ((uint64_t)first_sample + p->samples > 0xffffffffull) return fail(FW_ERR_BAD_ARG, "first_sample + samples overflows");
    if (p->pixel_ids) for (uint32_t i = 0; i < n_view; i++) if (p->pixel_ids[i] >= full) return fail(FW_ERR_BAD_ARG, "pixel id out of range");
    if (vg && (uint64_t)n_view * vg->n >= (1ull << 30)) return fail(FW_ERR_UNSUPPORTED, "too many pixels in one view group");
    const uint32_t n_pix = vg ? n_view * vg->n : n_view;
    const auto wall0 = std::chrono::steady_clock::now();
    HIPCHK(hipSetDevice(sc->device));
    hipStream_t stream = (hipStream_t)p->stream;
    Workspace *ws = workspace_for(sc->device);
    if (!ws) return fail(FW_ERR_OOM, "no workspace for this device");
    std::unique_lock<std::mutex> ws_guard(ws->mu, std::defer_lock);
    if (!rd) ws_guard.lock();
    { const int irc = init_device_locked(ws, sc->device); if (irc) return irc; }
    if (!rd) ws->kernels.clear();
    const bool dl = delta_lights(sc);
    if (dl && (p->flags & (FW_FLAG_ENV_SAMPLING | FW_FLAG_ALL_EMITTERS)))
        return fail(FW_ERR_UNSUPPORTED, "point, spot and directional lights do not combine with FW_FLAG_ENV_SAMPLING or FW_FLAG_ALL_EMITTERS");
    if (int erc = ensure_emitters(sc, p, ws)) return erc;
    if (int erc = ensure_env_dist(sc, p, ws)) return erc;
    const Options O = options();

    const BatchBudget bb = batch_budget(sc, p, O, ws->arena.bytes);
    int n_lanes = bb.n_lanes;
    const bool pl = all_emitters(sc, p);
    const bool ls_lights = !pl && light_sampling(sc, p), es = env_sampling(sc, p);
    const bool ls = ls_lights || es || pl || dl;
    const bool exact_product = bb.exact_product && !ls;
    const uint32_t budget = bb.budget;
    uint32_t spp_b = std::max<uint32_t>(1u, budget / n_pix);
    spp_b = std::min(spp_b, (p->samples + (uint32_t)n_lanes - 1) / (uint32_t)n_lanes);
    if (ri) spp_b = std::min(spp_b, (1u << 21) - 1u);
    uint64_t paths64 = (uint64_t)n_pix * spp_b;
    if (paths64 > 0x7fffffffull) return fail(FW_ERR_UNSUPPORTED, "too many paths per batch");
    uint32_t max_paths = (uint32_t)paths64;
    uint32_t n_batches = (p->samples + spp_b - 1) / spp_b;
    spp_b = (p->samples + n_batches - 1) / n_batches;
    max_paths = n_pix * spp_b;
    n_lanes = (int)std::min<uint32_t>((uint32_t)n_lanes, n_batches);
    if (vg && spp_b >= (1u << 21)) return fail(FW_ERR_UNSUPPORTED, "too many samples per batch for a view group");

    fw::DQueue q{};
    const uint32_t unit = (uint32_t)sc->n_cus * 4u * (p->use_bvh ? 20u : 28u);
    const uint64_t chunks = ((uint64_t)max_paths + 63u) / 64u;
    uint32_t want_waves = unit * (uint32_t)std::min<uint64_t>(3u, std::max<uint64_t>(1u, chunks / ((uint64_t)unit * 16u)));
    if (!p->use_bvh && n_lanes > 1) want_waves = chunks >= (1u << 20) ? unit : (uint32_t)sc->n_cus * 48u;
    if (O.waves > 0) want_waves = (uint32_t)O.waves;
    q.n_waves = std::max(4u, std::min(want_waves, (max_paths + 511u) / 512u));
    q.n_waves = (q.n_waves + 7u) & ~7u;
    uint32_t chunks_per_wave = (max_paths + q.n_waves * 64u - 1) / (q.n_waves * 64u);
    q.cpw_shift = 0;
    while ((1u << q.cpw_shift) < chunks_per_wave) q.cpw_shift++;
    q.cap = 64u << q.cpw_shift;
    uint64_t cap64 = (uint64_t)q.cap * q.n_waves;
    if (cap64 > 0x7fffffffull) return fail(FW_ERR_UNSUPPORTED, "too many path slots");
    uint32_t cap = (uint32_t)cap64;

#if FW_AB
    const bool fused_req = O.fused && !ls && !(p->use_bvh && sc->d.has_mesh) && !sc->has_ggx;
    const bool tlas_refill = !O.tlas_refill_off;
#else
    const bool fused_req = false, tlas_refill = true;
#endif
    const uint32_t exact_mode = fused_req ? 0u : ((sc->ex.mode & 1u) | (p->use_bvh ? (sc->ex.mode & 6u) | (ri ? fw::EX_TRACE_ZERO : 0u)
                                                                                   : ((sc->ex.mode & 4u) && sc->d.has_mesh ? 4u : 0u)));
    const bool park_meshes = p->use_bvh && sc->d.has_mesh != 0 && tlas_refill;
    const bool stage_rays = ri && ri->per_sample && !ri->on_device;
    int rc = FW_OK;
    auto need = [&](DevBuf &b, size_t n) { if (!rc) rc = b.alloc(n); };
    auto layout = [&](uint8_t *arena_base) -> size_t {
        size_t off = 0;
        auto put = [&](void *&dst, size_t n) { dst = arena_base ? arena_base + off : nullptr; off += (n + 255) & ~(size_t)255; };
        for (int l = 0; l < n_lanes; l++) {
            Workspace::Lane &L = ws->lanes[l];
            for (int k = 0; k < 2; k++) { put(L.ray_a[k], (size_t)cap * 16); put(L.ray_b[k], (size_t)cap * 8); put(L.state[k], (size_t)cap * 16); }
            put(L.hits, (size_t)cap * 8);
            put(L.sample_rad, (size_t)cap * 16);
            put(L.dep_bits, ((size_t)cap + 31) / 32 * 4);
            if (exact_product && !fused_req) put(L.atten, (size_t)cap * (fw::MAX_SEGMENTS - 1) * fw::B_ATTEN); else L.atten = nullptr;
            if (exact_mode) put(L.exact_slots, 2 * (size_t)max_paths * 4 + 64);
            put(L.wcount, (size_t)(fw::MAX_SEGMENTS + 1) * q.n_waves * 4);
            if (stage_rays) put(L.rays, (size_t)max_paths * 24); else L.rays = nullptr;
            if (ls) {
                put(L.s_ray_a, (size_t)cap * 16); put(L.s_ray_b, (size_t)cap * 8); put(L.s_state, (size_t)cap * 16); put(L.s_obj, (size_t)cap * 4);
                put(L.s_hits, (size_t)cap * 8); put(L.s_wcount, (size_t)(fw::MAX_SEGMENTS + 1) * q.n_waves * 4);
                put(L.pb[0], (size_t)cap * 4); put(L.pb[1], (size_t)cap * 4); put(L.nee, (size_t)cap * 16);
            }
            if (park_meshes) {
                const size_t pcap = (size_t)(q.cap + 64u) * q.n_waves;
                put(L.park_a, pcap * 16); put(L.park_b, pcap * 8); put(L.park_m, pcap * 16); put(L.pcount, (size_t)q.n_waves * 8);
            }
        }
        return off;
    };
    {
        size_t want = (layout(nullptr) + ((size_t)1 << 30) - 1) & ~(((size_t)1 << 30) - 1);
        if (want > ws->arena.bytes && ws->arena.bytes) want = std::max(want, (ws->arena.bytes + ws->arena.bytes / 4 + ((size_t)1 << 30) - 1) & ~(((size_t)1 << 30) - 1));
        const auto ta = std::chrono::steady_clock::now();
        const bool grow = want > ws->arena.bytes;
        if (!rc && grow) rc = arena_reserve_locked(ws, sc->device, want);
        if ((rd || ri) && grow) { ws->fg.key = 0; ws->fg.seen = 0; }
        if (O.trace && grow) fprintf(stderr, "[firework] render: path arena grown to %.1f GiB in %.2f ms\n", (double)want / (double)(1 << 30),
                                     std::chrono::duration<double, std::milli>(std::chrono::steady_clock::now() - ta).count());
        if (!rc) layout((uint8_t *)ws->arena.p);
    }
    for (int l = 0; l < n_lanes && !rc; l++)
        if (!ws->lanes[l].stream && n_lanes > 1) HIPCHK(hipStreamCreateWithFlags(&ws->lanes[l].stream, hipStreamNonBlocking));
    if (!rd) need(ws->accum, (size_t)n_pix * 16);
    need(ws->totals, (size_t)n_batches * fw::COUNT_STRIDE * 4);
    if (p->pixel_ids) need(ws->pixel_ids, (size_t)n_view * 4);
    const bool own_order = !p->pixel_ids && !user_accum && !rd && !ri && n_view >= 1024 && !O.no_tile_order;
    if (own_order) { const void *before = ws->tile_ids.p; need(ws->tile_ids, (size_t)n_view * 4); if (ws->tile_ids.p != before) ws->tile_w = ws->tile_h = 0; }
    if (vg) { need(ws->view_ids, (size_t)n_pix * 4); need(ws->view_cams, (size_t)vg->n * sizeof(fw::DCamera)); }
    const bool ray_table = ri && (ri->keys || ri->key_base != 0);
    if (ri) {
        need(ws->ray_err, 256);
        if (ray_table) need(ws->ray_keys, (size_t)n_pix * 4);
        if (!ri->per_sample && !ri->on_device) need(ws->ray_fixed, (size_t)n_pix * 24);
        const size_t host_bytes = ri->on_device ? 0 : ri->per_sample ? (size_t)n_lanes * max_paths * 24 : (size_t)n_pix * 24;
        if (!rc && ws->ray_host_bytes < host_bytes) {
            if (ws->ray_host) (void)hipHostFree(ws->ray_host);
            ws->ray_host = nullptr; ws->ray_host_bytes = 0;
            if (hipHostMalloc(&ws->ray_host, host_bytes, hipHostMallocDefault) != hipSuccess) return fail(FW_ERR_OOM, "pinned ray staging allocation failed");
            ws->ray_host_bytes = host_bytes;
        }
    }
    uint8_t *d_rgb8 = rgb8; float *d_gamma = gamma_rgb, *d_linear = linear_rgb;
    if (!p->outputs_on_device) {
        if (rgb8) { need(ws->out_rgb8, (size_t)n_pix * 3); d_rgb8 = (uint8_t *)ws->out_rgb8.p; }
        if (gamma_rgb) { need(ws->out_gamma, (size_t)n_pix * 12); d_gamma = (float *)ws->out_gamma.p; }
        if (linear_rgb) { need(ws->out_linear, (size_t)n_pix * 12); d_linear = (float *)ws->out_linear.p; }
    }
    if (rc) return rc;
    while (ws->events.size() < 3 + 2 * (size_t)n_batches) {
         hipEvent_t e; HIPCHK(hipEventCreateWithFlags(&e, ws->events.size() < 2 ? hipEventDefault : hipEventDisableTiming)); ws->events.push_back(e); }

    if (ws->ev_upload) HIPCHK(hipStreamWaitEvent(stream, ws->ev_upload, 0));
    if (p->pixel_ids) HIPCHK(hipMemcpyAsync(ws->pixel_ids.p, p->pixel_ids, (size_t)n_view * 4, hipMemcpyHostToDevice, stream));
    if (own_order && (ws->tile_w != p->width || ws->tile_h != p->height)) {
        ws->tile_w = ws->tile_h = 0;
        fw::launch_tile_order(stream, p->width, p->height, (uint32_t *)ws->tile_ids.p);
        ws->tile_w = p->width; ws->tile_h = p->height;
    }
    if (vg) {
        fw::launch_view_ids(stream, p->pixel_ids ? (const uint32_t *)ws->pixel_ids.p : (own_order ? (const uint32_t *)ws->tile_ids.p : nullptr), n_view, n_pix,
                            (uint32_t *)ws->view_ids.p);
        HIPCHK(hipMemcpyAsync(ws->view_cams.p, vg->cams, (size_t)vg->n * sizeof(fw::DCamera), hipMemcpyHostToDevice, stream));
    }
    if (ri) {
        HIPCHK(hipMemsetAsync(ws->ray_err.p, 0, 4, stream));
        if (ri->keys) HIPCHK(hipMemcpyAsync(ws->ray_keys.p, ri->keys, (size_t)n_pix * 4, ri->on_device ? hipMemcpyDeviceToDevice : hipMemcpyHostToDevice, stream));
        else if (ray_table) fw::launch_ray_keys(stream, ri->key_base, n_pix, (uint32_t *)ws->ray_keys.p);
        if (!ri->per_sample && !ri->on_device) {
            std::memcpy(ws->ray_host, ri->rays, (size_t)n_pix * 24);
            HIPCHK(hipMemcpyAsync(ws->ray_fixed.p, ws->ray_host, (size_t)n_pix * 24, hipMemcpyHostToDevice, stream));
        }
    }
    if (user_accum)
        HIPCHK(hipMemcpyAsync(ws->accum.p, user_accum, (size_t)n_pix * 16, p->outputs_on_device ? hipMemcpyDeviceToDevice : hipMemcpyHostToDevice, stream));
    else if (!rd) HIPCHK(hipMemsetAsync(ws->accum.p, 0, (size_t)n_pix * 16, stream));
    HIPCHK(hipMemsetAsync(ws->totals.p, 0, (size_t)n_batches * fw::COUNT_STRIDE * 4, stream));

    fw::LaunchCfg cfg{};
    set_walk_cfg(cfg, sc, O, q, p->use_bvh != 0, tlas_refill);
    cfg.log = &ws->kernels;
    int max_blocks = sc->n_cus * 8;
    cfg.blocks_other = (int)std::max<uint64_t>(1, std::min<uint64_t>(((uint64_t)n_pix + fw::BLOCK - 1) / fw::BLOCK, (uint64_t)max_blocks));
    cfg.shade_mode = !sc->has_expensive ? 1 : 0;
#if FW_AB
    if (O.no_shade_defer) cfg.shade_mode = 0; else if (sc->has_expensive && O.shade_list && q.cap <= 65536u && !sc->has_ggx) cfg.shade_mode = 2;
#endif
    cfg.gx = sc->has_ggx;

    fw::DCamera cam = vg ? vg->cams[0] : ri ? fw::DCamera{} : make_camera(p->camera, p->width, p->height);
    fw::DFrame fr{};
    fr.width = p->width; fr.height = p->height; fr.n_pixels = n_pix; fr.inv_n_pixels = 1.0f / (float)n_pix; fr.inv_width = 1.0f / (float)p->width;
    fr.pixel_ids = rd ? rd->ids : vg ? (const uint32_t *)ws->view_ids.p : ri ? (ray_table ? (const uint32_t *)ws->ray_keys.p : nullptr)
                 : (p->pixel_ids ? (const uint32_t *)ws->pixel_ids.p : (own_order ? (const uint32_t *)ws->tile_ids.p : nullptr));
    fr.scatter_out = own_order ? 1u : 0u;
    fr.seed32 = seed32_of(p->seed);
    fr.q_n_waves = q.n_waves; fr.q_shift = q.cpw_shift;
    fr.cam_pos[0] = cam.position[0]; fr.cam_pos[1] = cam.position[1]; fr.cam_pos[2] = cam.position[2];
    auto not_negative_zero = [](float x) { uint32_t b; std::memcpy(&b, &x, 4); return b != 0x80000000u; };
    bool one_position = true;
    if (vg) for (uint32_t v = 1; v < vg->n; v++) one_position = one_position && vg->cams[v].lens_radius == 0.f && std::memcmp(vg->cams[v].position, cam.position, sizeof cam.position) == 0;
    fr.pinhole0 = (!ri && one_position && cam.lens_radius == 0.f && not_negative_zero(cam.position[0]) && not_negative_zero(cam.position[1]) && not_negative_zero(cam.position[2]) &&
                   !O.no_short_rays) ? 1u : 0u;
    fr.hit4 = (!p->use_bvh && sc->simple_shapes && !exact_mode && !O.no_hit4 && !fused_req && !ls) ? 1u : 0u;
    const fw::DEnv &env = sc->d.env;
    fr.dep_pixel_major = (((n_pix <= 65536u && !O.dep_slot_major) || O.dep_pixel_major) && spp_b < (1u << 21)) ? 1u : 0u;
    fr.ex = sc->ex; fr.ex.mode = exact_mode;
    fr.chain_bits = (O.no_chain || fused_req || cfg.shade_mode == 2 || ls) ? 0u : sc->chain_bits;
    fr.skip_zero_deposits = (env.kind == 0 && env.color[0] == 0.f && env.color[1] == 0.f && env.color[2] == 0.f && !O.no_zero_skip && !ls) ? 1u : 0u;

    const bool timing = (p->flags & FW_FLAG_TIME_KERNELS) != 0;
    const bool count_deposits = (p->flags & FW_FLAG_COUNT_DEPOSITS) != 0 && fr.skip_zero_deposits != 0;
    const size_t per_batch_launches = 1 + 3 * fw::MAX_SEGMENTS + 2 + (ls ? 2 * (fw::MAX_SEGMENTS - 1) : 0);
    std::vector<std::vector<int>> ev_class(n_lanes);
    std::vector<size_t> ev_next(n_lanes, 0);
    if (timing) for (int l = 0; l < n_lanes; l++) {
        size_t want = 1 + per_batch_launches * ((n_batches + n_lanes - 1) / n_lanes);
        auto &ev = ws->lanes[l].events;
        while (ev.size() < want) { hipEvent_t e; HIPCHK(hipEventCreate(&e)); ev.push_back(e); }
    }
    const bool use_bvh = p->use_bvh != 0;
    const bool fused = fused_req;
#if FW_AB
    const bool stagger = n_lanes > 1 && O.stagger;
#else
    const bool stagger = false;
#endif

    const char *dump_file = O.dump_path.c_str();
    const bool dump_one = *dump_file && n_pix == 1 && p->samples == 1 && !fused;
    std::vector<float> dump_rec(dump_one ? (size_t)fw::MAX_SEGMENTS * 16 : 0, 0.f);

    HIPCHK(hipEventRecord(ws->events[0], stream));
    hipStream_t origin = stream;
    bool graph_replayed = false;
    auto fork_lanes = [&]() -> int {
        if (n_lanes > 1) {
            HIPCHK(hipEventRecord(ws->events[2], origin));
            for (int l = 0; l < n_lanes; l++) HIPCHK(hipStreamWaitEvent(ws->lanes[l].stream, ws->events[2], 0));
        }
        return FW_OK;
    };
    struct BatchCtx { fw::DFrame fr; fw::LaunchCfg cfg; fw::DPaths buf[2]; float2 *hits; float4 *srad; fw::DPark park; uint32_t *totals; uint32_t n_paths; int cur; int lane; hipStream_t ls;
                      fw::DShadow sh; fw::DEnvDist ed; fw::DEmitters em; fw::DDeltaLights dl; };
    constexpr uint64_t PHASE_LOCK_MIN_CHUNKS = 3u << 19;
    const bool phase_lock = n_lanes == 2 && !fused && (O.phase_lock == 1 || (O.phase_lock < 0 && !p->use_bvh && cfg.n_defer > 0 && chunks >= PHASE_LOCK_MIN_CHUNKS));
    std::vector<hipEvent_t> &pe = ws->phase_events;
    while (phase_lock && pe.size() < 2 * (size_t)fw::MAX_SEGMENTS) { hipEvent_t e; HIPCHK(hipEventCreateWithFlags(&e, hipEventDisableTiming)); pe.push_back(e); }
    float4 *const accum = rd ? rd->accum : (float4 *)ws->accum.p;
    auto begin_batch = [&](uint32_t b, BatchCtx &c) -> int {
        const int l = (int)(b % (uint32_t)n_lanes);
        Workspace::Lane &L = ws->lanes[l];
        c.lane = l; c.ls = n_lanes > 1 ? L.stream : origin;
        c.cfg = cfg; c.cfg.stream = c.ls; c.cfg.q.wcount = (uint32_t *)L.wcount;
        c.fr = fr;
        if (timing && ev_next[l] == 0) (void)hipEventRecord(L.events[0], c.ls);
        c.fr.sample0 = first_sample + b * spp_b;
        c.fr.dep_bits = (uint32_t *)L.dep_bits;
        c.fr.atten = (c.fr.chain_bits == 0 && exact_product && !fused_req) ? (float4 *)L.atten : nullptr; c.fr.atten_stride = cap;
        if (c.fr.skip_zero_deposits) HIPCHK(hipMemsetAsync(c.fr.dep_bits, 0, ((size_t)cap + 31) / 32 * 4, c.ls));
        if (exact_mode) {
            c.fr.ex.slots[0] = (uint32_t *)L.exact_slots; c.fr.ex.slots[1] = c.fr.ex.slots[0] + max_paths;
            c.fr.ex.count = c.fr.ex.slots[1] + max_paths; c.fr.ex.cap = max_paths;
            HIPCHK(hipMemsetAsync(c.fr.ex.count, 0, 64, c.ls));
        }
        c.fr.spp_batch = std::min(spp_b, p->samples - b * spp_b);
        c.n_paths = n_pix * c.fr.spp_batch;
        c.totals = (uint32_t *)ws->totals.p + (size_t)b * fw::COUNT_STRIDE;
        for (int k = 0; k < 2; k++) c.buf[k] = {(float4 *)L.ray_a[k], (float2 *)L.ray_b[k], (float4 *)L.state[k]};
        c.hits = (float2 *)L.hits;
        c.srad = (float4 *)L.sample_rad;
        c.park = fw::DPark{(float4 *)L.park_a, (float2 *)L.park_b, (float4 *)L.park_m, q.cap + 64u, (uint32_t *)L.pcount,
                           park_meshes ? (uint32_t *)L.pcount + q.n_waves : nullptr};
        if (park_meshes) HIPCHK(hipMemsetAsync(c.park.ptotal, 0, (size_t)q.n_waves * 4, c.ls));
        c.sh = fw::DShadow{}; c.ed = fw::DEnvDist{}; c.em = fw::DEmitters{}; c.dl = fw::DDeltaLights{};
        if (ls) {
            const float p_env = es ? ((ls_lights || pl) ? 0.5f : 1.f) : (dl ? (ls_lights ? 0.5f : 1.f) : 0.f);
            if (dl) c.dl = fw::DDeltaLights{(const float4 *)sc->dlights.p, sc->n_dlights, p_env};
            if (pl) c.em = emitters_of(sc, p_env);
            c.sh.lt = ls_lights ? fw::DLights{(const uint32_t *)sc->lights.p, sc->n_lights, (es || dl) ? (1.f - p_env) / (float)sc->n_lights : 1.f / (float)sc->n_lights}
                                : fw::DLights{(const uint32_t *)sc->lights.p, 0u, 0.f};
            if (es) c.ed = env_dist_of(sc->env_dist, sc->d.env, p_env);
            c.sh.ray_a = (float4 *)L.s_ray_a; c.sh.ray_b = (float2 *)L.s_ray_b; c.sh.state = (float4 *)L.s_state; c.sh.obj = (uint32_t *)L.s_obj;
            c.sh.wcount = (uint32_t *)L.s_wcount; c.sh.nee = (float4 *)L.nee;
            HIPCHK(hipMemsetAsync(c.sh.nee, 0, (size_t)cap * 16, c.ls));
        }
        c.cur = 0;
        return FW_OK;
    };
    auto timed = [&](BatchCtx &c, int cls, auto &&launch) {
        launch();
        if (timing) { (void)hipEventRecord(ws->lanes[c.lane].events[1 + ev_next[c.lane]], c.ls); ev_next[c.lane]++; ev_class[c.lane].push_back(cls); }
    };
    auto segment = [&](uint32_t b, BatchCtx &c, int seg, int which, int group_size) -> int {
#if FW_AB
        if (fused) { timed(c, 2, [&] { fw::launch_bounce(c.cfg, sc->d, c.fr, c.buf[c.cur], c.buf[c.cur ^ 1], c.srad, seg, use_bvh); }); c.cur ^= 1; return FW_OK; }
#endif
        if (stagger && seg == 0 && b > 0) HIPCHK(hipStreamWaitEvent(c.ls, ws->events[3 + n_batches + b - 1], 0));
        if (phase_lock && group_size == 2) {
// ... 16 lines not shown
            r[12] = (float)alive;
        }
        if (ls) {
            Workspace::Lane &L = ws->lanes[c.lane];
            c.sh.pb_in = (const float *)L.pb[c.cur]; c.sh.pb_out = (float *)L.pb[c.cur ^ 1];
            timed(c, 2, [&] { fw::launch_shade_nee(c.cfg, sc->d, c.fr, c.buf[c.cur], c.buf[c.cur ^ 1], c.hits, c.srad, seg, c.sh, es ? &c.ed : nullptr, pl ? &c.em : nullptr, dl ? &c.dl : nullptr); });
            if (seg < fw::MAX_SEGMENTS - 1) {
                fw::LaunchCfg scfg = c.cfg; scfg.q.wcount = c.sh.wcount;
                fw::DFrame sfr = c.fr; sfr.seed32 ^= fw::SHADOW_SEED; sfr.ex.mode = 0;
                const fw::DPaths sp{c.sh.ray_a, c.sh.ray_b, c.sh.state};
                timed(c, 1, [&] { fw::launch_extend(scfg, sc->d, sfr, sp, (float2 *)L.s_hits, seg + 1, use_bvh, c.park); });
                timed(c, 2, [&] { fw::launch_shadow_resolve(scfg, sc->d, c.sh, (const float2 *)L.s_hits, seg, es, pl, dl, c.srad); });
            }
        } else
        timed(c, 2, [&] { fw::launch_shade(c.cfg, sc->d, c.fr, c.buf[c.cur], c.buf[c.cur ^ 1], c.hits, c.srad, seg); });
        c.cur ^= 1;
        return FW_OK;
    };
    auto end_batch = [&](uint32_t b, BatchCtx &c) -> int {
        timed(c, 3, [&] { fw::launch_queue_totals(c.cfg, c.totals, c.park.ptotal); });
        if (count_deposits) fw::launch_count_deposits(c.cfg, c.fr.dep_bits, c.totals + 12);
        if (n_lanes > 1 && b > 0) HIPCHK(hipStreamWaitEvent(c.ls, ws->events[3 + b - 1], 0));
        if (rd) timed(c, 3, [&] { fw::launch_accumulate_adaptive(c.cfg, c.fr, c.srad, accum, rd->moments); });
        else timed(c, 3, [&] { fw::launch_accumulate(c.cfg, c.fr, c.srad, accum); });
        if (n_lanes > 1) HIPCHK(hipEventRecord(ws->events[3 + b], c.ls));
        return FW_OK;
    };
    auto batch_rays = [&](uint32_t b, const BatchCtx &c, const float *&src) -> int {
        if (!ri->per_sample) { src = ri->on_device ? ri->rays : (const float *)ws->ray_fixed.p; return FW_OK; }
        const size_t first = (size_t)b * spp_b * n_pix * 6, bytes = (size_t)c.n_paths * 24;
        if (ri->on_device) { src = ri->rays + first; return FW_OK; }
        HIPCHK(hipStreamSynchronize(c.ls));
        uint8_t *slab = (uint8_t *)ws->ray_host + (size_t)c.lane * max_paths * 24;
        std::memcpy(slab, ri->rays + first, bytes);
        HIPCHK(hipMemcpyAsync(ws->lanes[c.lane].rays, slab, bytes, hipMemcpyHostToDevice, c.ls));
        src = (const float *)ws->lanes[c.lane].rays;
        return FW_OK;
    };
    auto enqueue_frame = [&]() -> int {
    if (int frc = fork_lanes()) return frc;
    for (uint32_t b0 = 0; b0 < n_batches; b0 += (uint32_t)n_lanes) {
        const int group = (int)std::min<uint32_t>((uint32_t)n_lanes, n_batches - b0);
        BatchCtx ctx[Workspace::MAX_LANES];
        for (int g = 0; g < group; g++) {
            if (int brc = begin_batch(b0 + (uint32_t)g, ctx[g])) return brc;
            if (ri) {
                const float *src = nullptr;
                if (int src_rc = batch_rays(b0 + (uint32_t)g, ctx[g], src)) return src_rc;
                timed(ctx[g], 0, [&] { fw::launch_raygen_rays(ctx[g].cfg, src, ri->per_sample, (uint32_t *)ws->ray_err.p, ctx[g].fr, ctx[g].buf[0], ctx[g].n_paths); });
            }
            else if (vg) timed(ctx[g], 0, [&] { fw::launch_raygen_views(ctx[g].cfg, (const fw::DCamera *)ws->view_cams.p, n_view, ctx[g].fr, ctx[g].buf[0], ctx[g].srad, ctx[g].n_paths); });
            else timed(ctx[g], 0, [&] { fw::launch_raygen(ctx[g].cfg, cam, ctx[g].fr, ctx[g].buf[0], ctx[g].srad, ctx[g].n_paths); });
        }
        for (int seg = 0; seg < fw::MAX_SEGMENTS; seg++)
            for (int g = 0; g < group; g++)
                if (int src = segment(b0 + (uint32_t)g, ctx[g], seg, g, group)) return src;
        for (int g = 0; g < group; g++)
            if (int erc = end_batch(b0 + (uint32_t)g, ctx[g])) return erc;
        fr = ctx[group - 1].fr;
    }
    if (n_lanes > 1) HIPCHK(hipStreamWaitEvent(origin, ws->events[3 + n_batches - 1], 0));
    return FW_OK;
    };
    {
        Workspace::FrameGraph &fg = ws->fg;
        constexpr uint64_t GRAPH_MAX_CHUNKS = 1u << 19;
        const bool graph_ok = O.graph != 0 && !rd && !vg && !ri && !ls && !fg.broken && !timing && !dump_one && !phase_lock && !stagger && (O.graph == 1 || chunks < GRAPH_MAX_CHUNKS);
        uint64_t key = 0;
        if (graph_ok) {
            uint64_t h = 1469598103934665603ull;
            auto mix = [&](const void *ptr, size_t n) { const unsigned char *b = (const unsigned char *)ptr; for (size_t i = 0; i < n; i++) { h ^= b[i]; h *= 1099511628211ull; } };
            fw::LaunchCfg kc = cfg; kc.stream = nullptr;
            mix(&cam, sizeof cam); mix(&fr, sizeof fr); mix(&kc, sizeof kc); mix(&sc->d, sizeof sc->d); mix(&q, sizeof q);
            const uint64_t scalars[] = {n_batches, (uint64_t)n_lanes, spp_b, first_sample, p->samples, n_pix, max_paths, cap, exact_mode, (uint64_t)park_meshes, (uint64_t)phase_lock,
                                        (uint64_t)count_deposits, (uint64_t)exact_product, (uint64_t)use_bvh, (uint64_t)fused, (uint64_t)stagger, (uint64_t)(uintptr_t)accum, (uint64_t)(uintptr_t)ws->totals.p,
                                        (uint64_t)(uintptr_t)ws->arena.p, (uint64_t)ws->arena.bytes};
            mix(scalars, sizeof scalars);
            for (int l = 0; l < n_lanes; l++) { const Workspace::Lane &L = ws->lanes[l]; const void *ptrs[] = {L.ray_a[0], L.ray_a[1], L.ray_b[0], L.ray_b[1], L.state[0], L.state[1], L.hits, L.sample_rad, L.wcount, L.park_a, L.park_b, L.park_m, L.pcount, L.dep_bits, L.exact_slots, L.atten}; mix(ptrs, sizeof ptrs); }
            key = h | 1ull;
        }
        bool done = false;
        if (graph_ok && fg.exec && fg.key == key) {
            HIPCHK(hipGraphLaunch(fg.exec, stream));
            fr = fg.fr_after; done = true; graph_replayed = true;
            ws->kernels.merge(fg.kernels);
        } else if (graph_ok && fg.seen == key) {
            if (!fg.origin && hipStreamCreateWithFlags(&fg.origin, hipStreamNonBlocking) != hipSuccess) { fg.origin = nullptr; fg.broken = true; }
            if (!fg.broken && hipStreamBeginCapture(fg.origin, hipStreamCaptureModeRelaxed) == hipSuccess) {
                origin = fg.origin;
                if (O.trace) fprintf(stderr, "[firework] GRAPH: capturing (%u batches, %d lanes, phase lock %d)\n", n_batches, n_lanes, (int)phase_lock);
                const fw::KernelLog before = ws->kernels;
                ws->kernels.clear();
                const int crc = enqueue_frame();
                fg.kernels = ws->kernels;
                ws->kernels.merge(before);
                origin = stream;
                hipGraph_t g = nullptr;
                const hipError_t ee = hipStreamEndCapture(fg.origin, &g);
                if (O.trace) fprintf(stderr, "[firework] GRAPH: capture ended: enqueue %d, end %s\n", crc, hipGetErrorString(ee));
                if (fg.exec) { (void)hipGraphExecDestroy(fg.exec); fg.exec = nullptr; fg.key = 0; }
                if (crc == FW_OK && ee == hipSuccess && g && hipGraphInstantiate(&fg.exec, g, nullptr, nullptr, 0) == hipSuccess) {
                    fg.key = key; fg.fr_after = fr;
                    (void)hipGraphDestroy(g);
                    if (O.trace) fprintf(stderr, "[firework] GRAPH: instantiated\n");
                    HIPCHK(hipGraphLaunch(fg.exec, stream));
                    if (O.trace) fprintf(stderr, "[firework] GRAPH: launched\n");
                    graph_replayed = true;
                    done = true;
                } else {
                    if (g) (void)hipGraphDestroy(g);
                    fg.exec = nullptr; fg.broken = true; (void)hipGetLastError();
                    if (O.trace) fprintf(stderr, "[firework] GRAPH: capture failed (%d, %s): frames run as plain launches from here on\n", crc, hipGetErrorString(ee));
                }
            } else { fg.broken = true; (void)hipGetLastError(); }
        }
        if (graph_ok) fg.seen = key;
        if (!done) { if (int frc = enqueue_frame()) return frc; }
    }
    cfg.stream = stream;
    if (vg) fw::launch_resolve_views(cfg, fr, n_view, (const float4 *)ws->accum.p, p->samples, p->gamma, d_rgb8, d_gamma, d_linear);
    else if (!rd) fw::launch_resolve(cfg, fr, (const float4 *)ws->accum.p, first_sample + p->samples, p->gamma, d_rgb8, d_gamma, d_linear);
    if (user_accum) HIPCHK(hipMemcpyAsync(user_accum, ws->accum.p, (size_t)n_pix * 16, p->outputs_on_device ? hipMemcpyDeviceToDevice : hipMemcpyDeviceToHost, stream));
    HIPCHK(hipEventRecord(ws->events[1], stream));
    HIPCHK(hipGetLastError());

    if (dump_one) {
        if (FILE *fp = fopen(dump_file, "wb")) {
// ... 3123 lines not shown
    catch (...) { return fail(FW_ERR_BAD_ARG, "unexpected exception in fw_selftest_bvh_build"); }
}

int fw_selftest_bvh_trees(int device, const float *boxes, uint32_t n, float *ref_nodes, float *sah_nodes, uint32_t stats[4]) {
    if (!boxes || n == 0 || !ref_nodes || !sah_nodes || !stats || device < -1 || n > fw::NODE_MASK) return fail(FW_ERR_BAD_ARG, "bad argument");
    try {
        FlatBvh ref, sah;
        if (device >= 0) {
            int ndev = 0;
            if (hipGetDeviceCount(&ndev) != hipSuccess || ndev <= 0) { (void)hipGetLastError(); return fail(FW_ERR_NO_DEVICE, "no HIP device visible"); }
            if (device >= ndev) return fail(FW_ERR_BAD_ARG, "device index out of range");
            HIPCHK(hipSetDevice(device));
            std::string msg;
            int rc = fw::device_build_tree(device, fw::BUILD_MEDIAN, boxes, n, ref.nodes, ref.depth, nullptr, msg);
            if (!rc) rc = fw::device_build_tree(device, fw::BUILD_SAH, boxes, n, sah.nodes, sah.depth, nullptr, msg);
            if (rc) return fail(rc, msg);
        } else {
            std::vector<Box> b(n);
            for (uint32_t i = 0; i < n; i++) b[i] = Box{{boxes[6 * i], boxes[6 * i + 1], boxes[6 * i + 2]}, {boxes[6 * i + 3], boxes[6 * i + 4], boxes[6 * i + 5]}};
            if (int rc = build_tree(-1, fw::BUILD_MEDIAN, b, ref, nullptr, nullptr)) return rc;
            if (int rc = build_tree(-1, fw::BUILD_SAH, b, sah, nullptr, nullptr)) return rc;
        }
        if (ref.count() > 2 * (size_t)n - 1 || sah.count() > 2 * (size_t)n - 1) return fail(FW_ERR_HIP, "tree larger than 2n - 1 nodes");
        std::memcpy(ref_nodes, ref.nodes.data(), ref.nodes.size() * 4);
        std::memcpy(sah_nodes, sah.nodes.data(), sah.nodes.size() * 4);
        stats[0] = ref.count(); stats[1] = ref.depth; stats[2] = sah.count(); stats[3] = sah.depth;
        return FW_OK;
    }
    catch (std::bad_alloc &) { return fail(FW_ERR_OOM, "host allocation failed"); }
    catch (...) { return fail(FW_ERR_BAD_ARG, "unexpected exception in fw_selftest_bvh_trees"); }
}

#if FW_AB
int fw_debug_ab(void) { return 1; }
#endif

int fw_debug_kernels(int device, char *buf, uint32_t cap) {
    try {
        if (device < -1 || device >= MAX_DEVICES) return fail(FW_ERR_BAD_ARG, "fw_debug_kernels: device out of range");
        if (!buf && cap > 0) return fail(FW_ERR_BAD_ARG, "fw_debug_kernels: null buffer with cap > 0");
        std::vector<std::string> names;
        if (device < 0) for (uint32_t i = 0; i < fw::KID_COUNT; i++) names.push_back(fw::KERNEL_NAMES[i]);
        else {
            Workspace *ws = workspace_for(device);
            if (!ws) return fail(FW_ERR_OOM, "no workspace for this device");
            fw::KernelLog log;
            { std::lock_guard<std::mutex> g(ws->mu); log = ws->kernels; }
            for (uint32_t i = 0; i < fw::KID_COUNT; i++) {
                if (!log.has(i)) continue;
                if (fw::KERNEL_FAMILY[i] < 0) { names.push_back(fw::KERNEL_NAMES[i]); continue; }
                const uint32_t waves[3] = {16u, 12u, 8u};
                for (int b = 0; b < 3; b++) if (log.waves[i] & (1u << b)) names.push_back(std::string(fw::KERNEL_NAMES[i]) + "@" + std::to_string(waves[b]));
            }
        }
        std::sort(names.begin(), names.end());
        std::string all;
        for (const std::string &n : names) { if (!all.empty()) all += ','; all += n; }
        if (cap > 0) { const size_t k = std::min<size_t>(all.size(), (size_t)cap - 1); std::memcpy(buf, all.data(), k); buf[k] = 0; }
        return (int)all.size();
    }
    catch (std::bad_alloc &) { return fail(FW_ERR_OOM, "host allocation failed"); }
    catch (...) { return fail(FW_ERR_BAD_ARG, "unexpected exception in fw_debug_kernels"); }
}

int fw_init(int device, uint64_t arena_bytes) {
    try {
        if (int rc = use_device(device)) return rc;
        Workspace *ws = workspace_for(device);
        if (!ws) return fail(FW_ERR_OOM, "no workspace for this device");
        std::lock_guard<std::mutex> g(ws->mu);
        int rc = init_device_locked(ws, device);
        if (rc) return rc;
        size_t want = arena_bytes == FW_INIT_NO_ARENA ? 0 : (arena_bytes ? (size_t)arena_bytes : default_arena_bytes(ws));
        want = (want + ((size_t)1 << 20) - 1) & ~(((size_t)1 << 20) - 1);
        if (want > ws->arena.bytes) {
            const auto ta = std::chrono::steady_clock::now();
            rc = arena_reserve_locked(ws, device, want);
            if (options().trace) fprintf(stderr, "[firework] fw_init: path arena of %.1f GiB in %.2f ms\n", (double)want / (double)(1 << 30),
                                         std::chrono::duration<double, std::milli>(std::chrono::steady_clock::now() - ta).count());
        }
        return rc;
    }
    catch (std::bad_alloc &) { return fail(FW_ERR_OOM, "host allocation failed"); }
    catch (...) { return fail(FW_ERR_BAD_ARG, "unexpected exception in fw_init"); }
}

int fw_scene_create(const fw_scene_desc *desc, int device, fw_scene **out) {
    try { return create_scene_impl(desc, device, out); }
    catch (std::bad_alloc &) { return fail(FW_ERR_OOM, "host allocation failed"); }
    catch (...) { return fail(FW_ERR_BAD_ARG, "unexpected exception in fw_scene_create"); }
}

int fw_scene_update(fw_scene *scene, const fw_scene_desc *desc) {
    try { return update_scene_impl(scene, desc); }
    catch (std::bad_alloc &) { return fail(FW_ERR_OOM, "host allocation failed"); }
    catch (...) { return fail(FW_ERR_BAD_ARG, "unexpected exception in fw_scene_update"); }
}

int fw_scene_set_lights(fw_scene *scene, const fw_light *lights, uint32_t n) {
    try { return set_lights_impl(scene, lights, n); }
    catch (std::bad_alloc &) { return fail(FW_ERR_OOM, "host allocation failed"); }
    catch (...) { return fail(FW_ERR_BAD_ARG, "unexpected exception in fw_scene_set_lights"); }
}

int fw_check_lights(const fw_light *lights, uint32_t n) {
    try { return check_lights_impl(lights, n); }
// ... 633 lines not shown
```

Before: 43390 Mrays/s.

## Fuse all path segments into a single persistent extend+shade kernel launch

Moves the extend (deferred-object intersection) and shade bodies into shared include files so that a new fused kernel can run every bounce segment inside one launch, in place of separate extend and shade launches per segment. This targets per-segment launch overhead and the inter-kernel gaps between bounces. It also adds a load_obj overload that reads scene objects through the constant address space, which may give scalar loads. The cost is a heavier fused kernel with more register and LDS pressure, and the launch path now depends on can_fuse_segments.

```diff
diff --git a/firework_amd/csrc/fw_device.h b/firework_amd/csrc/fw_device.h
--- a/firework_amd/csrc/fw_device.h
+++ b/firework_amd/csrc/fw_device.h
@@ -302,10 +302,11 @@
 struct KernelLog {
     uint64_t bits[(KID_COUNT + 63) / 64];
     uint8_t waves[KID_COUNT];
+    uint8_t fused;
     void clear() { *this = KernelLog{}; }
     void add(KernelId id) { bits[id >> 6] |= 1ull << (id & 63u); }
     void add(KernelId id, uint32_t w) { add(id); waves[id] |= (uint8_t)(w == 16u ? 1u : w == 12u ? 2u : 4u); }
-    void merge(const KernelLog &o) { for (size_t i = 0; i < sizeof bits / sizeof bits[0]; i++) bits[i] |= o.bits[i]; for (uint32_t i = 0; i < KID_COUNT; i++) waves[i] |= o.waves[i]; }
+    void merge(const KernelLog &o) { for (size_t i = 0; i < sizeof bits / sizeof bits[0]; i++) bits[i] |= o.bits[i]; for (uint32_t i = 0; i < KID_COUNT; i++) waves[i] |= o.waves[i]; fused |= o.fused; }
     bool has(uint32_t id) const { return ((bits[id >> 6] >> (id & 63u)) & 1u) != 0; }
 };
 
@@ -348,6 +349,9 @@
 void launch_extend_exact(const LaunchCfg &, const DScene &, const DFrame &, const DPaths &in, float2 *hits, int segment, bool use_bvh);
 void launch_shade(const LaunchCfg &, const DScene &, const DFrame &, DPaths in, DPaths out, const float2 *hits,
                   float4 *sample_rad, int segment);
+bool can_fuse_segments(const LaunchCfg &, const DScene &);
+void launch_segments(const LaunchCfg &, const DScene &, const DFrame &, DPaths in, DPaths out, float2 *hits, float4 *sample_rad, int first, int last);
+extern const char *const FUSED_KERNEL_NAMES[4];
 void launch_shade_nee(const LaunchCfg &, const DScene &, const DFrame &, DPaths in, DPaths out, const float2 *hits,
                       float4 *sample_rad, int segment, const DShadow &, const DEnvDist *ed, const DEmitters *em, const DDeltaLights *dl = nullptr);
 void launch_shadow_resolve(const LaunchCfg &, const DScene &, const DShadow &, const float2 *hits, int segment, bool env, bool pl, bool dl = false,
diff --git a/firework_amd/csrc/fw_extend_defer.inc b/firework_amd/csrc/fw_extend_defer.inc
--- /dev/null
+++ b/firework_amd/csrc/fw_extend_defer.inc
@@ -0,0 +1,91 @@
+    const float TMIN = 0.001f, TMAX = 2e9f;
+    const uint32_t n_first = sc.n_objects - n_def;
+    uint32_t cnt0 = 0, cnt1 = 0;
+    const RngKey nokey{0, 0, 0};
+    auto write_final = [&](uint32_t slot, float t, uint32_t code) {
+        if (f.hit4) reinterpret_cast<uint32_t *>(hits)[slot] = code; else qst(&hits[slot], make_float2(t, __uint_as_float(code)));
+    };
+    auto put = [&](uint32_t *L, uint32_t e, uint32_t sb, float t, uint32_t code, const Ray &r) {
+        L[e] = sb; L[64u + e] = __float_as_uint(t); L[128u + e] = code;
+        L[192u + e] = __float_as_uint(r.o.x); L[256u + e] = __float_as_uint(r.o.y); L[320u + e] = __float_as_uint(r.o.z);
+        L[384u + e] = __float_as_uint(r.d.x); L[448u + e] = __float_as_uint(r.d.y); L[512u + e] = __float_as_uint(r.d.z);
+    };
+    auto get = [&](const uint32_t *L, uint32_t e, uint32_t &sb, float &t, uint32_t &code, Ray &r) {
+        sb = L[e]; t = __uint_as_float(L[64u + e]); code = L[128u + e];
+        r.o = mk(__uint_as_float(L[192u + e]), __uint_as_float(L[256u + e]), __uint_as_float(L[320u + e]));
+        r.d = mk(__uint_as_float(L[384u + e]), __uint_as_float(L[448u + e]), __uint_as_float(L[512u + e]));
+    };
+    auto test = [&](uint32_t d, const Ray &r, float &t, uint32_t &code) {
+        const uint32_t k = n_first + d;
+        const Obj o = load_obj(scan_objs, k);
+        float tt; uint32_t prim;
+        if (hit_rect3d(o.q3, o.q4, to_object_space(o, r), TMIN, t, tt, prim)) { t = tt; code = (k << sc.prim_bits) | prim; }
+    };
+    auto append = [&](uint32_t *L, uint32_t &cnt, bool want, uint32_t sb, float t, uint32_t code, const Ray &r) {
+        const unsigned long long m = __ballot(want);
+        if (!m) return;
+        const uint32_t rank = __builtin_amdgcn_mbcnt_hi((uint32_t)(m >> 32), __builtin_amdgcn_mbcnt_lo((uint32_t)m, 0u));
+        if (want) put(L, cnt + rank, sb, t, code, r);
+        cnt += (uint32_t)__popcll(m);
+    };
+    auto make_room = [&](uint32_t need0, uint32_t need1) {
+        const bool r0 = cnt0 != 0u && cnt0 + need0 > 64u;
+        const uint32_t pass_on = r0 ? (uint32_t)__popcll(__ballot(lane < cnt0 && (L0[lane] >> 31) != 0u)) : 0u;
+#pragma nounroll
+        for (int phase = 0; phase < 2; phase++) {
+            const bool r1 = cnt1 != 0u && (phase == 0 ? cnt1 + pass_on > 64u : cnt1 + need1 > 64u);
+            if (r1) {
+                uint32_t sb = 0, code = MISS; float t = TMAX; Ray r{mk(0, 0, 0), mk(0, 0, 1)};
+                if (lane < cnt1) { get(L1, lane, sb, t, code, r); test(1, r, t, code); write_final(sb, t, code); }
+                cnt1 = 0;
+            }
+            if (phase == 0 && r0) {
+                uint32_t sb = 0, code = MISS; float t = TMAX; Ray r{mk(0, 0, 0), mk(0, 0, 1)};
+                const bool on = lane < cnt0;
+                if (on) { get(L0, lane, sb, t, code, r); test(0, r, t, code); }
+                cnt0 = 0;
+                const bool more = on && (sb >> 31) != 0u;
+                const uint32_t slot = sb & 0x7fffffffu;
+                if (on && !more) write_final(slot, t, code);
+                append(L1, cnt1, more, slot, t, code, r);
+            }
+        }
+    };
+    float4 ra_n = make_float4(0, 0, 0, 0); float2 rb_n = make_float2(0, 0);
+    if (lane < n) { ra_n = qld(&in.ray_a[base + lane]); rb_n = load_ray_b(in, base + lane, f, segment); }
+    for (uint32_t c0 = 0; c0 < n; c0 += 64u) {
+        const uint32_t j = c0 + lane, i = base + j;
+        const float4 ra = ra_n; const float2 rb = rb_n;
+        if (j + 64u < n) { ra_n = qld(&in.ray_a[i + 64u]); rb_n = load_ray_b(in, i + 64u, f, segment); }
+        const bool active = j < n;
+        float best_t = TMAX; uint32_t best_obj = MISS, best_prim = 0;
+        bool may0 = false, may1 = false;
+        const Ray r = make_ray(ra, rb, f, segment);
+        if (active) {
+            auto op = scan_objs;
+            const Rcp rcx = make_rcp(r.d.x), rcy = make_rcp(r.d.y), rcz = make_rcp(r.d.z);
+            for (uint32_t k = 0; k < n_first; k++, op += OBJ_Q) {
+                const Obj o = load_obj(op, 0);
+                float t; uint32_t prim = 0; bool h;
+                const uint32_t kind = obj_kind(o);
+                if (kind >= 1u && kind <= 3u && !(obj_flags(o) & OF_ROTATED) && o.q4.y == 0.f) {
+                    const Ray ro{r.o - mk(o.q0.w, o.q1.w, o.q2.w), r.d};
+                    if (kind == 1u) h = hit_rect_rcp<0>(o.q3.x, o.q3.y, o.q3.z, o.q3.w, o.q4.x, ro, rcz, TMIN, best_t, t);
+                    else if (kind == 2u) h = hit_rect_rcp<1>(o.q3.x, o.q3.y, o.q3.z, o.q3.w, o.q4.x, ro, rcy, TMIN, best_t, t);
+                    else h = hit_rect_rcp<2>(o.q3.x, o.q3.y, o.q3.z, o.q3.w, o.q4.x, ro, rcx, TMIN, best_t, t);
+                } else h = hit_object<false, 0, false, SIMPLE>(sc, o, k, r, TMIN, best_t, nullptr, nokey, segment, t, prim);
+                if (h) { best_t = t; best_obj = k; best_prim = prim; }
+            }
+            const fwpt::RayTerms rt = fwpt::ray_terms(r.o.x, r.o.y, r.o.z, rcx.r, rcy.r, rcz.r);
+            const auto cb = scan_cull + 2 * ((size_t)sc.n_objects + n_first);
+            may0 = fwpt::pretest_fma(rt, cb[0].x, cb[0].y, cb[0].z, cb[1].x, cb[1].y, cb[1].z, best_t);
+            if (n_def > 1u) may1 = fwpt::pretest_fma(rt, cb[2].x, cb[2].y, cb[2].z, cb[3].x, cb[3].y, cb[3].z, best_t);
+        }
+        const uint32_t code = best_obj == MISS ? MISS : ((best_obj << sc.prim_bits) | best_prim);
+        const bool c1 = may1 && !may0;
+        make_room((uint32_t)__popcll(__ballot(may0)), (uint32_t)__popcll(__ballot(c1)));
+        if (active && !may0 && !may1) write_final(i, best_t, code);
+        append(L0, cnt0, may0, i | (may1 ? 0x80000000u : 0u), best_t, code, r);
+        append(L1, cnt1, c1, i, best_t, code, r);
+    }
+    make_room(65u, 65u);
diff --git a/firework_amd/csrc/fw_kernels.hip b/firework_amd/csrc/fw_kernels.hip
--- a/firework_amd/csrc/fw_kernels.hip
+++ b/firework_amd/csrc/fw_kernels.hip
@@ -401,6 +401,23 @@
 
 __device__ __forceinline__ Obj load_obj(const float4 *__restrict__ objs, uint32_t j) {
     const float4 *p = objs + (size_t)j * OBJ_Q;
+    float4 r0 = p[0], r3 = p[3], r4 = p[4], r5 = p[5];
+    Obj o;
+    o.q0 = make_float4(r3.x, r3.y, r3.z, r0.x); o.q1 = make_float4(r4.x, r4.y, r4.z, r0.y); o.q2 = make_float4(r5.x, r5.y, r5.z, r0.z);
+    o.q3 = p[1]; o.q4 = p[2];
+    o.kf = __float_as_uint(r0.w); o.material = __float_as_uint(r3.w);
+    o.aux0 = __float_as_uint(r4.w); o.aux1 = __float_as_uint(r5.w);
+    return o;
+}
+struct ConstQuads {
+    const __attribute__((address_space(4))) f4v *p;
+    __device__ __forceinline__ float4 operator[](size_t i) const { const f4v v = p[i]; return make_float4(v.x, v.y, v.z, v.w); }
+    __device__ __forceinline__ ConstQuads operator+(size_t n) const { return ConstQuads{p + n}; }
+    __device__ __forceinline__ ConstQuads &operator+=(size_t n) { p += n; return *this; }
+};
+__device__ __forceinline__ ConstQuads const_quads(const float4 *q) { return ConstQuads{(const __attribute__((address_space(4))) f4v *)q}; }
+__device__ __forceinline__ Obj load_obj(ConstQuads objs, uint32_t j) {
+    const ConstQuads p = objs + (size_t)j * OBJ_Q;
     float4 r0 = p[0], r3 = p[3], r4 = p[4], r5 = p[5];
     Obj o;
     o.q0 = make_float4(r3.x, r3.y, r3.z, r0.x); o.q1 = make_float4(r4.x, r4.y, r4.z, r0.y); o.q2 = make_float4(r5.x, r5.y, r5.z, r0.z);
@@ -1374,98 +1391,9 @@
     const uint32_t w = wave_index(), lane = threadIdx.x & 63u;
     if (w >= q.n_waves) return;
     const uint32_t n = q.wcount[(size_t)segment * q.n_waves + w], base = w * q.cap;
-    const float TMIN = 0.001f, TMAX = 2e9f;
-    const uint32_t n_first = sc.n_objects - n_def;
     uint32_t *const L0 = lds_defer, *const L1 = lds_defer + DEFER_FIELDS * 64u;
-    uint32_t cnt0 = 0, cnt1 = 0;
-    const RngKey nokey{0, 0, 0};
-    auto write_final = [&](uint32_t slot, float t, uint32_t code) {
-        if (f.hit4) reinterpret_cast<uint32_t *>(hits)[slot] = code; else qst(&hits[slot], make_float2(t, __uint_as_float(code)));
-    };
-    auto put = [&](uint32_t *L, uint32_t e, uint32_t sb, float t, uint32_t code, const Ray &r) {
-        L[e] = sb; L[64u + e] = __float_as_uint(t); L[128u + e] = code;
-        L[192u + e] = __float_as_uint(r.o.x); L[256u + e] = __float_as_uint(r.o.y); L[320u + e] = __float_as_uint(r.o.z);
-        L[384u + e] = __float_as_uint(r.d.x); L[448u + e] = __float_as_uint(r.d.y); L[512u + e] = __float_as_uint(r.d.z);
-    };
-    auto get = [&](const uint32_t *L, uint32_t e, uint32_t &sb, float &t, uint32_t &code, Ray &r) {
-        sb = L[e]; t = __uint_as_float(L[64u + e]); code = L[128u + e];
-        r.o = mk(__uint_as_float(L[192u + e]), __uint_as_float(L[256u + e]), __uint_as_float(L[320u + e]));
-        r.d = mk(__uint_as_float(L[384u + e]), __uint_as_float(L[448u + e]), __uint_as_float(L[512u + e]));
-    };
-    auto test = [&](uint32_t d, const Ray &r, float &t, uint32_t &code) {
-        const uint32_t k = n_first + d;
-        const Obj o = load_obj(sc.obj, k);
-        float tt; uint32_t prim;
-        if (hit_rect3d(o.q3, o.q4, to_object_space(o, r), TMIN, t, tt, prim)) { t = tt; code = (k << sc.prim_bits) | prim; }
-    };
-    auto append = [&](uint32_t *L, uint32_t &cnt, bool want, uint32_t sb, float t, uint32_t code, const Ray &r) {
-        const unsigned long long m = __ballot(want);
-        if (!m) return;
-        const uint32_t rank = __builtin_amdgcn_mbcnt_hi((uint32_t)(m >> 32), __builtin_amdgcn_mbcnt_lo((uint32_t)m, 0u));
-        if (want) put(L, cnt + rank, sb, t, code, r);
-        cnt += (uint32_t)__popcll(m);
-    };
-    auto make_room = [&](uint32_t need0, uint32_t need1) {
-        const bool r0 = cnt0 != 0u && cnt0 + need0 > 64u;
-        const uint32_t pass_on = r0 ? (uint32_t)__popcll(__ballot(lane < cnt0 && (L0[lane] >> 31) != 0u)) : 0u;
-#pragma nounroll
-        for (int phase = 0; phase < 2; phase++) {
-            const bool r1 = cnt1 != 0u && (phase == 0 ? cnt1 + pass_on > 64u : cnt1 + need1 > 64u);
-            if (r1) {
-                uint32_t sb = 0, code = MISS; float t = TMAX; Ray r{mk(0, 0, 0), mk(0, 0, 1)};
-                if (lane < cnt1) { get(L1, lane, sb, t, code, r); test(1, r, t, code); write_final(sb, t, code); }
-                cnt1 = 0;
-            }
-            if (phase == 0 && r0) {
-                uint32_t sb = 0, code = MISS; float t = TMAX; Ray r{mk(0, 0, 0), mk(0, 0, 1)};
-                const bool on = lane < cnt0;
-                if (on) { get(L0, lane, sb, t, code, r); test(0, r, t, code); }
-                cnt0 = 0;
-                const bool more = on && (sb >> 31) != 0u;
-                const uint32_t slot = sb & 0x7fffffffu;
-                if (on && !more) write_final(slot, t, code);
-                append(L1, cnt1, more, slot, t, code, r);
-            }
-        }
-    };
-    float4 ra_n = make_float4(0, 0, 0, 0); float2 rb_n = make_float2(0, 0);
-    if (lane < n) { ra_n = qld(&in.ray_a[base + lane]); rb_n = load_ray_b(in, base + lane, f, segment); }
-    for (uint32_t c0 = 0; c0 < n; c0 += 64u) {
-        const uint32_t j = c0 + lane, i = base + j;
-        const float4 ra = ra_n; const float2 rb = rb_n;
-        if (j + 64u < n) { ra_n = qld(&in.ray_a[i + 64u]); rb_n = load_ray_b(in, i + 64u, f, segment); }
-        const bool active = j < n;
-        float best_t = TMAX; uint32_t best_obj = MISS, best_prim = 0;
-        bool may0 = false, may1 = false;
-        const Ray r = make_ray(ra, rb, f, segment);
-        if (active) {
-            const float4 *op = sc.obj;
-            const Rcp rcx = make_rcp(r.d.x), rcy = make_rcp(r.d.y), rcz = make_rcp(r.d.z);
-            for (uint32_t k = 0; k < n_first; k++, op += OBJ_Q) {
-                const Obj o = load_obj(op, 0);
-                float t; uint32_t prim = 0; bool h;
-                const uint32_t kind = obj_kind(o);
-                if (kind >= 1u && kind <= 3u && !(obj_flags(o) & OF_ROTATED) && o.q4.y == 0.f) {
-                    const Ray ro{r.o - mk(o.q0.w, o.q1.w, o.q2.w), r.d};
-                    if (kind == 1u) h = hit_rect_rcp<0>(o.q3.x, o.q3.y, o.q3.z, o.q3.w, o.q4.x, ro, rcz, TMIN, best_t, t);
-                    else if (kind == 2u) h = hit_rect_rcp<1>(o.q3.x, o.q3.y, o.q3.z, o.q3.w, o.q4.x, ro, rcy, TMIN, best_t, t);
-                    else h = hit_rect_rcp<2>(o.q3.x, o.q3.y, o.q3.z, o.q3.w, o.q4.x, ro, rcx, TMIN, best_t, t);
-                } else h = hit_object<false, 0, false, SIMPLE>(sc, o, k, r, TMIN, best_t, nullptr, nokey, segment, t, prim);
-                if (h) { best_t = t; best_obj = k; best_prim = prim; }
-            }
-            const fwpt::RayTerms rt = fwpt::ray_terms(r.o.x, r.o.y, r.o.z, rcx.r, rcy.r, rcz.r);
-            const float4 *const cb = sc.obj_cull + 2 * ((size_t)sc.n_objects + n_first);
-            may0 = fwpt::pretest_fma(rt, cb[0].x, cb[0].y, cb[0].z, cb[1].x, cb[1].y, cb[1].z, best_t);
-            if (n_def > 1u) may1 = fwpt::pretest_fma(rt, cb[2].x, cb[2].y, cb[2].z, cb[3].x, cb[3].y, cb[3].z, best_t);
-        }
-        const uint32_t code = best_obj == MISS ? MISS : ((best_obj << sc.prim_bits) | best_prim);
-        const bool c1 = may1 && !may0;
-        make_room((uint32_t)__popcll(__ballot(may0)), (uint32_t)__popcll(__ballot(c1)));
-        if (active && !may0 && !may1) write_final(i, best_t, code);
-        append(L0, cnt0, may0, i | (may1 ? 0x80000000u : 0u), best_t, code, r);
-        append(L1, cnt1, c1, i, best_t, code, r);
-    }
-    make_room(65u, 65u);
+    const float4 *const scan_objs = sc.obj, *const scan_cull = sc.obj_cull;
+#include "fw_extend_defer.inc"
 }
 
 __global__ __launch_bounds__(WB) __attribute__((amdgpu_waves_per_eu(7, 8)))
@@ -3026,116 +2954,52 @@
     const uint32_t n = q.wcount[(size_t)segment * q.n_waves + w];
     const uint32_t base = w * q.cap;
     uint32_t out_n = 0;
-    uint32_t list_n = 0;
-    PH_DECL;
-    auto compact = [&](bool alive, const Ray &nr, V3 nbeta, uint32_t nchain, uint32_t path_id, uint32_t c0 = 0xffffffffu) {
-        const unsigned long long mask = __ballot(alive);
-        const uint32_t rank = __builtin_amdgcn_mbcnt_hi((uint32_t)(mask >> 32), __builtin_amdgcn_mbcnt_lo((uint32_t)mask, 0u));
-#if FW_SHADE_STATIC_STORES
-        if (c0 != 0xffffffffu) {
-#if FW_SHADE_STATIC_STORES == 2
-            const uint32_t dst = base + (alive ? out_n + rank : q.cap - 1u);
-#else
-            const uint32_t dst = base + (alive ? out_n + rank : min(c0 + 64u + lane, q.cap - 1u));
-#endif
-            qst(&out.ray_a[dst], make_float4(nr.o.x, nr.o.y, nr.o.z, nr.d.x));
-            qst(&out.ray_b[dst], make_float2(nr.d.y, nr.d.z));
-            if (CHAIN) qst(&reinterpret_cast<float2 *>(out.state)[dst], make_float2(__uint_as_float(nchain), __uint_as_float(path_id)));
-            else qst(&out.state[dst], make_float4(nbeta.x, nbeta.y, nbeta.z, __uint_as_float(path_id)));
-        } else
-#endif
-        if (alive) {
-            const uint32_t dst = base + out_n + rank;
-            qst(&out.ray_a[dst], make_float4(nr.o.x, nr.o.y, nr.o.z, nr.d.x));
-            qst(&out.ray_b[dst], make_float2(nr.d.y, nr.d.z));
-            if (CHAIN) qst(&reinterpret_cast<float2 *>(out.state)[dst], make_float2(__uint_as_float(nchain), __uint_as_float(path_id)));
-            else qst(&out.state[dst], make_float4(nbeta.x, nbeta.y, nbeta.z, __uint_as_float(path_id)));
-        }
-        if (f.ex.mode)
-            flag_exact(f.ex, alive && needs_exact(f.ex, nr.o.x, nr.o.y, nr.o.z, nr.d.x, nr.d.y, nr.d.z), base + out_n + rank, segment + 1);
-        out_n += (uint32_t)__popcll(mask);
-    };
-    auto load_st = [&](uint32_t idx) { return CHAIN ? load_state_chain(in, idx, segment) : load_state(in, idx, segment); };
-    auto load_hit = [&](uint32_t idx) { return f.hit4 ? make_float2(0.f, __uint_as_float(reinterpret_cast<const uint32_t *>(hits)[idx])) : qld(&hits[idx]); };
-    auto run_list = [&](uint32_t take) {
-        bool alive = false;
-        Ray nr{mk(0, 0, 0), mk(0, 0, 0)}; V3 nbeta = mk(0, 0, 0); uint32_t path_id = 0, nchain = 0;
-        if (lane < take) {
-            const uint32_t i = base + shade_list[list_n - take + lane];
-            const float4 ra = qld(&in.ray_a[i]), st = load_st(i); const float2 rb = load_ray_b(in, i, f, segment), hr = load_hit(i);
-            path_id = __float_as_uint(st.w);
-            alive = shade_path<false, CHAIN>(sc, f, objp, matp, texp, make_ray(ra, rb, f, segment), mk(st.x, st.y, st.z), __float_as_uint(st.x), path_id, hr.x, __float_as_uint(hr.y), segment, sample_rad, nr, nbeta, nchain PH_PASS);
-        }
-        list_n -= take;
-        compact(alive, nr, nbeta, nchain, path_id);
-    };
-    float4 ra_n = make_float4(0, 0, 0, 0), st_n = ra_n; float2 rb_n = make_float2(0, 0), hr_n = rb_n;
-#if FW_SHADE_PIPE
-    auto prefetch = [&](uint32_t jn) {
-        const uint32_t in_ = base + jn;
-        ra_n = qld(&in.ray_a[in_]);
-        rb_n = qld(&in.ray_b[short_rays(f, segment) ? base : in_]);
-        if (CHAIN) { const float2 v = qld(&reinterpret_cast<const float2 *>(in.state)[segment == 0 ? base : in_]); st_n = make_float4(v.x, 0.f, 0.f, v.y); }
-        else st_n = qld(&in.state[segment == 0 ? base : in_]);
-        hr_n = load_hit(in_);
-    };
-    auto fix_implicit = [&](float4 &st_, float2 &rb_, uint32_t slot) {
-        if (segment == 0) st_ = CHAIN ? make_float4(0.f, 0.f, 0.f, __uint_as_float(slot)) : make_float4(1.f, 1.f, 1.f, __uint_as_float(slot));
-        if (short_rays(f, segment)) rb_ = make_float2(0.f, 0.f);
-    };
-    if (n) {
-        prefetch(min(lane, n - 1u));
-        const uint32_t d0 = base + lane;
-        qst(&out.ray_a[d0], make_float4(0.f, 0.f, 0.f, 0.f));
-        qst(&out.ray_b[d0], make_float2(0.f, 0.f));
-        if (CHAIN) qst(&reinterpret_cast<float2 *>(out.state)[d0], make_float2(0.f, 0.f)); else qst(&out.state[d0], make_float4(0.f, 0.f, 0.f, 0.f));
-    }
-#else
-    if (lane < n) { ra_n = qld(&in.ray_a[base + lane]); rb_n = load_ray_b(in, base + lane, f, segment); st_n = load_st(base + lane); hr_n = load_hit(base + lane); }
-#endif
-    for (uint32_t c0 = 0; c0 < n; c0 += 64u) {
-        const uint32_t j = c0 + lane;
-        const uint32_t i = base + j;
-        float4 ra = ra_n, st = st_n; float2 rb = rb_n, hr = hr_n;
-#if FW_SHADE_PIPE
-        fix_implicit(st, rb, i);
-        const RngKey key_ = key_of(f, __float_as_uint(st.w));
-        prefetch(min(j + 64u, n - 1u));
-        const RngKey *pre_key = &key_;
-#else
-        if (j + 64u < n) { ra_n = qld(&in.ray_a[i + 64u]); rb_n = load_ray_b(in, i + 64u, f, segment); st_n = load_st(i + 64u); hr_n = load_hit(i + 64u); }
-        const RngKey *pre_key = nullptr;
-#endif
-        bool alive = false, later = false;
-        Ray nr{mk(0, 0, 0), mk(0, 0, 0)}; V3 nbeta = mk(0, 0, 0); uint32_t path_id = 0, nchain = 0;
-        if (j < n) {
-            PH_T0;
-            Ray r = make_ray(ra, rb, f, segment);
-            V3 beta = mk(st.x, st.y, st.z);
-            path_id = __float_as_uint(st.w);
-            const uint32_t hit_code = __float_as_uint(hr.y);
-#ifdef FW_ABL_SHADE_COPY
-            alive = hit_code != MISS && segment < 10; nr = r; nbeta = beta; nchain = __float_as_uint(st.x) + (pre_key ? pre_key->pixel & 1u : 0u);
-#else
-            if (MODE == 2 && expensive_shading(sc, objp, matp, hit_code)) later = true;
-            else alive = shade_path<MODE != 0, CHAIN>(sc, f, objp, matp, texp, r, beta, __float_as_uint(st.x), path_id, hr.x, hit_code, segment, sample_rad, nr, nbeta, nchain PH_PASS, pre_key);
-#endif
-            PH_ADD(0);
-        }
-        { PH_T0; compact(alive, nr, nbeta, nchain, path_id, c0); PH_ADD(7); }
-        if (MODE == 2) {
-            const unsigned long long lm = __ballot(later);
-            if (lm) {
-                const uint32_t lr = __builtin_amdgcn_mbcnt_hi((uint32_t)(lm >> 32), __builtin_amdgcn_mbcnt_lo((uint32_t)lm, 0u));
-                if (later) shade_list[list_n + lr] = (uint16_t)j;
-                list_n += (uint32_t)__popcll(lm);
-                if (list_n >= 64u) run_list(64u);
-            }
-        }
-    }
-    if (MODE == 2) while (list_n) run_list(min(list_n, 64u));
+#include "fw_shade_body.inc"
     if (lane == 0) q.wcount[(size_t)(segment + 1) * q.n_waves + w] = out_n;
     PH_FLUSH(1);
+}
+
+template <bool SIMPLE, bool CHAIN>
+__global__ __launch_bounds__(WB) __attribute__((amdgpu_waves_per_eu(6, 8)))
+void k_segments_boxlist(DScene sc, DFrame f, DPaths in, DPaths out, float2 *hits, float4 *sample_rad, DQueue q, int first, int last,
+                        uint32_t n_def, uint32_t n_mat, uint32_t n_tex, uint32_t table_quads) {
+    constexpr int LDS_TAB = 1, MODE = 1;
+    const uint32_t w = __builtin_amdgcn_readfirstlane(wave_index()), lane0 = threadIdx.x & 63u;
+    uint16_t *const shade_list = nullptr;
+#include "fw_shade_tables.inc"
+    if (w >= q.n_waves) return;
+    uint32_t *const L0 = reinterpret_cast<uint32_t *>(lds_tables + table_quads), *const L1 = L0 + DEFER_FIELDS * 64u;
+    const uint32_t base0 = w * q.cap;
+#define FW_PHASE_IDS uint32_t lane = lane0, base = base0; asm volatile("" : "+v"(lane), "+s"(base))
+    uint32_t n = q.wcount[(size_t)first * q.n_waves + w];
+    auto phase_end = [] {
+        asm volatile("s_waitcnt vmcnt(0)" ::: "memory");
+        __builtin_amdgcn_fence(__ATOMIC_RELEASE, "workgroup");
+        __builtin_amdgcn_fence(__ATOMIC_ACQUIRE, "workgroup");
+    };
+#pragma nounroll
+    for (int segment = first; segment <= last; segment++) {
+        if (n == 0u) {
+            if (lane0 == 0) for (int s = segment; s <= last; s++) q.wcount[(size_t)(s + 1) * q.n_waves + w] = 0u;
+            return;
+        }
+        {
+            FW_PHASE_IDS;
+            const ConstQuads scan_objs = const_quads(sc.obj), scan_cull = const_quads(sc.obj_cull);
+#include "fw_extend_defer.inc"
+        }
+        phase_end();
+        uint32_t out_n = 0;
+        {
+            FW_PHASE_IDS;
+#include "fw_shade_body.inc"
+        }
+        if (lane0 == 0) q.wcount[(size_t)(segment + 1) * q.n_waves + w] = out_n;
+        phase_end();
+        const DPaths t = in; in = out; out = t;
+        n = out_n;
+    }
+#undef FW_PHASE_IDS
 }
 template <int LDS_TAB, int MODE>
 __attribute__((amdgpu_waves_per_eu(FW_SHADE_WAVES, 8)))
@@ -3912,6 +3776,7 @@
     FW_KERNEL_IDS(FW_KID_NAME)
 #undef FW_KID_NAME
 };
+const char *const FUSED_KERNEL_NAMES[4] = {"k_segments_boxlist<false,no chain>", "k_segments_boxlist<false,chain>", "k_segments_boxlist<true,no chain>", "k_segments_boxlist<true,chain>"};
 const signed char KERNEL_FAMILY[KID_COUNT] = {
 #define FW_KID_FAM(id, name, fam) fam,
     FW_KERNEL_IDS(FW_KID_FAM)
@@ -4041,6 +3906,24 @@
 #undef FW_SHADE_C
 #undef FW_SHADE
 }
+bool can_fuse_segments(const LaunchCfg &c, const DScene &sc) {
+    return c.n_defer > 0 && !c.gx && c.shade_mode == 1 && shade_tables(c, sc).lt == 1;
+}
+void launch_segments(const LaunchCfg &c, const DScene &sc, const DFrame &f, DPaths in, DPaths out, float2 *hits, float4 *sample_rad, int first, int last) {
+    const ShadeTables t = shade_tables(c, sc);
+    const size_t lds = t.lds + (size_t)2 * 64 * DEFER_FIELDS * 4;
+    const uint32_t tq = (uint32_t)(t.lds / sizeof(float4));
+    const bool chain = f.chain_bits != 0;
+    if (c.log) {
+        c.log->add(c.simple_set ? KID_EXTEND_LINEAR_DEFER_S : KID_EXTEND_LINEAR_DEFER_N);
+        c.log->add(chain ? KID_SHADE_111 : KID_SHADE_110);
+        c.log->fused |= (uint8_t)(1u << ((c.simple_set ? 2u : 0u) | (chain ? 1u : 0u)));
+    }
+#define FW_SEGMENTS(S, C) hipLaunchKernelGGL((k_segments_boxlist<S, C>), wave_grid(c), dim3(WB), lds, c.stream, sc, f, in, out, hits, sample_rad, c.q, first, last, c.n_defer, c.n_mat, c.n_tex, tq)
+    if (c.simple_set) { if (chain) FW_SEGMENTS(true, true); else FW_SEGMENTS(true, false); }
+    else { if (chain) FW_SEGMENTS(false, true); else FW_SEGMENTS(false, false); }
+#undef FW_SEGMENTS
+}
 void launch_shade_nee(const LaunchCfg &c, const DScene &sc, const DFrame &f, DPaths in, DPaths out, const float2 *hits,
                       float4 *sample_rad, int segment, const DShadow &sh, const DEnvDist *ed, const DEmitters *em, const DDeltaLights *dl) {
     const ShadeTables t = shade_tables(c, sc);
@@ -4113,6 +3996,7 @@
     FW_TOUCH((k_shade<0, 0, false>)); FW_TOUCH((k_shade<0, 0, true>)); FW_TOUCH((k_shade<0, 1, false>)); FW_TOUCH((k_shade<0, 1, true>));
     FW_TOUCH((k_shade<1, 0, false>)); FW_TOUCH((k_shade<1, 0, true>)); FW_TOUCH((k_shade<1, 1, false>)); FW_TOUCH((k_shade<1, 1, true>));
     FW_TOUCH((k_shade<2, 0, false>)); FW_TOUCH((k_shade<2, 0, true>)); FW_TOUCH((k_shade<2, 1, false>)); FW_TOUCH((k_shade<2, 1, true>));
+    FW_TOUCH((k_segments_boxlist<true, true>)); FW_TOUCH((k_segments_boxlist<true, false>)); FW_TOUCH((k_segments_boxlist<false, true>)); FW_TOUCH((k_segments_boxlist<false, false>));
 #undef FW_TOUCH
     (void)hipGetLastError();
 }
diff --git a/firework_amd/csrc/fw_runtime.cpp b/firework_amd/csrc/fw_runtime.cpp
--- a/firework_amd/csrc/fw_runtime.cpp
+++ b/firework_amd/csrc/fw_runtime.cpp
@@ -53,6 +53,7 @@
     double wide_node_cost = 0.0005;
     int wide = -1;
     int build = -1;
+    int fuse_segments = -1;
     long waves = 0;
     long long paths_per_batch = 0;
     std::string dump_path;
@@ -62,7 +63,7 @@
 #endif
 };
 const char *const OPTION_NAMES[] = {"BVH", "NO_EXACT", "EXACT_ALL", "EXACT_FORM", "NO_DEFER", "NO_HIT4", "NO_HOIST", "NO_LDS_TABLES", "NO_LDS_TREES", "NO_LDS_TRIS",
-                                    "NO_SHORT_RAYS", "NO_TILE_ORDER", "NO_ZERO_SKIP", "DEP_PIXEL_MAJOR", "DEP_SLOT_MAJOR", "NO_CHAIN", "EXACT_PRODUCT", "PHASE_LOCK", "GRAPH", "SOFT_SHEAR_LOG2", "EXACT_SHEAR_LOG2", "EXACT_FAR_X", "WIDE_NODE_COST", "TRACE", "STREAMS", "WIDE", "BUILD", "WAVES",
+                                    "NO_SHORT_RAYS", "NO_TILE_ORDER", "NO_ZERO_SKIP", "DEP_PIXEL_MAJOR", "DEP_SLOT_MAJOR", "NO_CHAIN", "EXACT_PRODUCT", "PHASE_LOCK", "FUSE_SEGMENTS", "GRAPH", "SOFT_SHEAR_LOG2", "EXACT_SHEAR_LOG2", "EXACT_FAR_X", "WIDE_NODE_COST", "TRACE", "STREAMS", "WIDE", "BUILD", "WAVES",
                                     "PATHS_PER_BATCH", "DUMP_PATH",
 #if FW_AB
                                     "FUSED", "TLAS_REFILL", "SHADE_LIST", "NO_SHADE_DEFER", "STAGGER", "DEBUG_WIDE_LEVELS",
@@ -90,6 +91,7 @@
     else if (n == "NO_CHAIN") o.no_chain = on();
     else if (n == "EXACT_PRODUCT") o.exact_product = v && atoi(v) != 0;
     else if (n == "PHASE_LOCK") o.phase_lock = v ? (atoi(v) != 0 ? 1 : 0) : -1;
+    else if (n == "FUSE_SEGMENTS") o.fuse_segments = v ? (atoi(v) != 0 ? 1 : 0) : -1;
     else if (n == "GRAPH") o.graph = v ? (atoi(v) != 0 ? 1 : 0) : -1;
     else if (n == "SOFT_SHEAR_LOG2") o.soft_shear_log2 = v ? (int)num() : 5;
     else if (n == "EXACT_SHEAR_LOG2") o.exact_shear_log2 = v ? (int)num() : 10;
@@ -1938,6 +1940,15 @@
     return (uint32_t)std::max<uint64_t>(budget, 1u << 16);
 }
 
+static int frame_shade_mode(const fw_scene *sc, const Options &O, uint32_t cap) {
+    int mode = !sc->has_expensive ? 1 : 0;
+#if FW_AB
+    if (O.no_shade_defer) mode = 0; else if (sc->has_expensive && O.shade_list && cap <= 65536u && !sc->has_ggx) mode = 2;
+#else
+    (void)O; (void)cap;
+#endif
+    return mode;
+}
 void set_walk_cfg(fw::LaunchCfg &cfg, const fw_scene *sc, const Options &O, const fw::DQueue &q, bool use_bvh, bool tlas_refill) {
     cfg.q = q;
     cfg.tlas_depth = (int)sc->tlas_depth; cfg.blas_depth = (int)sc->blas_depth;
@@ -2156,11 +2167,38 @@
     n_lanes = (int)std::min<uint32_t>((uint32_t)n_lanes, n_batches);
     if (vg && spp_b >= (1u << 21)) return fail(FW_ERR_UNSUPPORTED, "too many samples per batch for a view group");
 
+#if FW_AB
+    const bool fused_req = O.fused && !ls && !(p->use_bvh && sc->d.has_mesh) && !sc->has_ggx;
+    const bool tlas_refill = !O.tlas_refill_off;
+#else
+    const bool fused_req = false, tlas_refill = true;
+#endif
+    const uint32_t exact_mode = fused_req ? 0u : ((sc->ex.mode & 1u) | (p->use_bvh ? (sc->ex.mode & 6u) | (ri ? fw::EX_TRACE_ZERO : 0u)
+                                                                                   : ((sc->ex.mode & 4u) && sc->d.has_mesh ? 4u : 0u)));
+    const bool timing = (p->flags & FW_FLAG_TIME_KERNELS) != 0;
+#if FW_AB
+    const bool stagger = n_lanes > 1 && O.stagger;
+#else
+    const bool stagger = false;
+#endif
+    const char *dump_file = O.dump_path.c_str();
+    const bool dump_one = *dump_file && n_pix == 1 && p->samples == 1 && !fused_req;
+    fw::LaunchCfg cfg{};
+    {
+        fw::DQueue none{};
+        set_walk_cfg(cfg, sc, O, none, p->use_bvh != 0, tlas_refill);
+        cfg.shade_mode = frame_shade_mode(sc, O, 0u); cfg.gx = sc->has_ggx;
+    }
+    const bool fuse_segments = O.fuse_segments == 1 && !p->use_bvh && exact_mode == 0 && !ls && !fused_req && !stagger && !timing && !dump_one &&
+                               fw::can_fuse_segments(cfg, sc->d);
     fw::DQueue q{};
+    constexpr uint64_t BIG_BATCH_CHUNKS = 1u << 20;
     const uint32_t unit = (uint32_t)sc->n_cus * 4u * (p->use_bvh ? 20u : 28u);
     const uint64_t chunks = ((uint64_t)max_paths + 63u) / 64u;
     uint32_t want_waves = unit * (uint32_t)std::min<uint64_t>(3u, std::max<uint64_t>(1u, chunks / ((uint64_t)unit * 16u)));
-    if (!p->use_bvh && n_lanes > 1) want_waves = chunks >= (1u << 20) ? unit : (uint32_t)sc->n_cus * 48u;
+    if (!p->use_bvh && n_lanes > 1) want_waves = chunks >= BIG_BATCH_CHUNKS ? unit : (uint32_t)sc->n_cus * 48u;
+    if (!p->use_bvh && n_lanes > 1 && chunks >= BIG_BATCH_CHUNKS && cfg.n_defer > 0 && cfg.shade_mode == 1 && !ls) want_waves = 2u * unit;
+    if (fuse_segments && chunks >= BIG_BATCH_CHUNKS) want_waves = 4u * unit;
     if (O.waves > 0) want_waves = (uint32_t)O.waves;
     q.n_waves = std::max(4u, std::min(want_waves, (max_paths + 511u) / 512u));
     q.n_waves = (q.n_waves + 7u) & ~7u;
@@ -2172,14 +2210,6 @@
     if (cap64 > 0x7fffffffull) return fail(FW_ERR_UNSUPPORTED, "too many path slots");
     uint32_t cap = (uint32_t)cap64;
 
-#if FW_AB
-    const bool fused_req = O.fused && !ls && !(p->use_bvh && sc->d.has_mesh) && !sc->has_ggx;
-    const bool tlas_refill = !O.tlas_refill_off;
-#else
-    const bool fused_req = false, tlas_refill = true;
-#endif
-    const uint32_t exact_mode = fused_req ? 0u : ((sc->ex.mode & 1u) | (p->use_bvh ? (sc->ex.mode & 6u) | (ri ? fw::EX_TRACE_ZERO : 0u)
-                                                                                   : ((sc->ex.mode & 4u) && sc->d.has_mesh ? 4u : 0u)));
     const bool park_meshes = p->use_bvh && sc->d.has_mesh != 0 && tlas_refill;
     const bool stage_rays = ri && ri->per_sample && !ri->on_device;
     int rc = FW_OK;
@@ -2277,15 +2307,11 @@
     else if (!rd) HIPCHK(hipMemsetAsync(ws->accum.p, 0, (size_t)n_pix * 16, stream));
     HIPCHK(hipMemsetAsync(ws->totals.p, 0, (size_t)n_batches * fw::COUNT_STRIDE * 4, stream));
 
-    fw::LaunchCfg cfg{};
     set_walk_cfg(cfg, sc, O, q, p->use_bvh != 0, tlas_refill);
     cfg.log = &ws->kernels;
     int max_blocks = sc->n_cus * 8;
     cfg.blocks_other = (int)std::max<uint64_t>(1, std::min<uint64_t>(((uint64_t)n_pix + fw::BLOCK - 1) / fw::BLOCK, (uint64_t)max_blocks));
-    cfg.shade_mode = !sc->has_expensive ? 1 : 0;
-#if FW_AB
-    if (O.no_shade_defer) cfg.shade_mode = 0; else if (sc->has_expensive && O.shade_list && q.cap <= 65536u && !sc->has_ggx) cfg.shade_mode = 2;
-#endif
+    cfg.shade_mode = frame_shade_mode(sc, O, q.cap);
     cfg.gx = sc->has_ggx;
 
     fw::DCamera cam = vg ? vg->cams[0] : ri ? fw::DCamera{} : make_camera(p->camera, p->width, p->height);
@@ -2309,7 +2335,6 @@
     fr.chain_bits = (O.no_chain || fused_req || cfg.shade_mode == 2 || ls) ? 0u : sc->chain_bits;
     fr.skip_zero_deposits = (env.kind == 0 && env.color[0] == 0.f && env.color[1] == 0.f && env.color[2] == 0.f && !O.no_zero_skip && !ls) ? 1u : 0u;
 
-    const bool timing = (p->flags & FW_FLAG_TIME_KERNELS) != 0;
     const bool count_deposits = (p->flags & FW_FLAG_COUNT_DEPOSITS) != 0 && fr.skip_zero_deposits != 0;
     const size_t per_batch_launches = 1 + 3 * fw::MAX_SEGMENTS + 2 + (ls ? 2 * (fw::MAX_SEGMENTS - 1) : 0);
     std::vector<std::vector<int>> ev_class(n_lanes);
@@ -2321,14 +2346,6 @@
     }
     const bool use_bvh = p->use_bvh != 0;
     const bool fused = fused_req;
-#if FW_AB
-    const bool stagger = n_lanes > 1 && O.stagger;
-#else
-    const bool stagger = false;
-#endif
-
-    const char *dump_file = O.dump_path.c_str();
-    const bool dump_one = *dump_file && n_pix == 1 && p->samples == 1 && !fused;
     std::vector<float> dump_rec(dump_one ? (size_t)fw::MAX_SEGMENTS * 16 : 0, 0.f);
 
     HIPCHK(hipEventRecord(ws->events[0], stream));
@@ -2344,7 +2361,7 @@
     struct BatchCtx { fw::DFrame fr; fw::LaunchCfg cfg; fw::DPaths buf[2]; float2 *hits; float4 *srad; fw::DPark park; uint32_t *totals; uint32_t n_paths; int cur; int lane; hipStream_t ls;
                       fw::DShadow sh; fw::DEnvDist ed; fw::DEmitters em; fw::DDeltaLights dl; };
     constexpr uint64_t PHASE_LOCK_MIN_CHUNKS = 3u << 19;
-    const bool phase_lock = n_lanes == 2 && !fused && (O.phase_lock == 1 || (O.phase_lock < 0 && !p->use_bvh && cfg.n_defer > 0 && chunks >= PHASE_LOCK_MIN_CHUNKS));
+    const bool phase_lock = !fuse_segments && n_lanes == 2 && !fused && (O.phase_lock == 1 || (O.phase_lock < 0 && !p->use_bvh && cfg.n_defer > 0 && chunks >= PHASE_LOCK_MIN_CHUNKS));
     std::vector<hipEvent_t> &pe = ws->phase_events;
     while (phase_lock && pe.size() < 2 * (size_t)fw::MAX_SEGMENTS) { hipEvent_t e; HIPCHK(hipEventCreateWithFlags(&e, hipEventDisableTiming)); pe.push_back(e); }
     float4 *const accum = rd ? rd->accum : (float4 *)ws->accum.p;
@@ -2467,6 +2484,13 @@
             else if (vg) timed(ctx[g], 0, [&] { fw::launch_raygen_views(ctx[g].cfg, (const fw::DCamera *)ws->view_cams.p, n_view, ctx[g].fr, ctx[g].buf[0], ctx[g].srad, ctx[g].n_paths); });
             else timed(ctx[g], 0, [&] { fw::launch_raygen(ctx[g].cfg, cam, ctx[g].fr, ctx[g].buf[0], ctx[g].srad, ctx[g].n_paths); });
         }
+        if (fuse_segments)
+            for (int g = 0; g < group; g++) {
+                BatchCtx &c = ctx[g];
+                fw::launch_segments(c.cfg, sc->d, c.fr, c.buf[0], c.buf[1], c.hits, c.srad, 0, fw::MAX_SEGMENTS - 1);
+                c.cur = fw::MAX_SEGMENTS & 1;
+            }
+        else
         for (int seg = 0; seg < fw::MAX_SEGMENTS; seg++)
             for (int g = 0; g < group; g++)
                 if (int src = segment(b0 + (uint32_t)g, ctx[g], seg, g, group)) return src;
@@ -2487,7 +2511,7 @@
             auto mix = [&](const void *ptr, size_t n) { const unsigned char *b = (const unsigned char *)ptr; for (size_t i = 0; i < n; i++) { h ^= b[i]; h *= 1099511628211ull; } };
             fw::LaunchCfg kc = cfg; kc.stream = nullptr;
             mix(&cam, sizeof cam); mix(&fr, sizeof fr); mix(&kc, sizeof kc); mix(&sc->d, sizeof sc->d); mix(&q, sizeof q);
-            const uint64_t scalars[] = {n_batches, (uint64_t)n_lanes, spp_b, first_sample, p->samples, n_pix, max_paths, cap, exact_mode, (uint64_t)park_meshes, (uint64_t)phase_lock,
+            const uint64_t scalars[] = {n_batches, (uint64_t)n_lanes, spp_b, first_sample, p->samples, n_pix, max_paths, cap, exact_mode, (uint64_t)park_meshes, (uint64_t)phase_lock, (uint64_t)fuse_segments,
                                         (uint64_t)count_deposits, (uint64_t)exact_product, (uint64_t)use_bvh, (uint64_t)fused, (uint64_t)stagger, (uint64_t)(uintptr_t)accum, (uint64_t)(uintptr_t)ws->totals.p,
                                         (uint64_t)(uintptr_t)ws->arena.p, (uint64_t)ws->arena.bytes};
             mix(scalars, sizeof scalars);
@@ -5717,6 +5741,7 @@
                 const uint32_t waves[3] = {16u, 12u, 8u};
                 for (int b = 0; b < 3; b++) if (log.waves[i] & (1u << b)) names.push_back(std::string(fw::KERNEL_NAMES[i]) + "@" + std::to_string(waves[b]));
             }
+            for (int b = 0; b < 4; b++) if (log.fused & (1u << b)) names.push_back(fw::FUSED_KERNEL_NAMES[b]);
         }
         std::sort(names.begin(), names.end());
         std::string all;
diff --git a/firework_amd/csrc/fw_shade_body.inc b/firework_amd/csrc/fw_shade_body.inc
--- /dev/null
+++ b/firework_amd/csrc/fw_shade_body.inc
@@ -0,0 +1,108 @@
+    uint32_t list_n = 0;
+    PH_DECL;
+    auto compact = [&](bool alive, const Ray &nr, V3 nbeta, uint32_t nchain, uint32_t path_id, uint32_t c0 = 0xffffffffu) {
+        const unsigned long long mask = __ballot(alive);
+        const uint32_t rank = __builtin_amdgcn_mbcnt_hi((uint32_t)(mask >> 32), __builtin_amdgcn_mbcnt_lo((uint32_t)mask, 0u));
+#if FW_SHADE_STATIC_STORES
+        if (c0 != 0xffffffffu) {
+#if FW_SHADE_STATIC_STORES == 2
+            const uint32_t dst = base + (alive ? out_n + rank : q.cap - 1u);
+#else
+            const uint32_t dst = base + (alive ? out_n + rank : min(c0 + 64u + lane, q.cap - 1u));
+#endif
+            qst(&out.ray_a[dst], make_float4(nr.o.x, nr.o.y, nr.o.z, nr.d.x));
+            qst(&out.ray_b[dst], make_float2(nr.d.y, nr.d.z));
+            if (CHAIN) qst(&reinterpret_cast<float2 *>(out.state)[dst], make_float2(__uint_as_float(nchain), __uint_as_float(path_id)));
+            else qst(&out.state[dst], make_float4(nbeta.x, nbeta.y, nbeta.z, __uint_as_float(path_id)));
+        } else
+#endif
+        if (alive) {
+            const uint32_t dst = base + out_n + rank;
+            qst(&out.ray_a[dst], make_float4(nr.o.x, nr.o.y, nr.o.z, nr.d.x));
+            qst(&out.ray_b[dst], make_float2(nr.d.y, nr.d.z));
+            if (CHAIN) qst(&reinterpret_cast<float2 *>(out.state)[dst], make_float2(__uint_as_float(nchain), __uint_as_float(path_id)));
+            else qst(&out.state[dst], make_float4(nbeta.x, nbeta.y, nbeta.z, __uint_as_float(path_id)));
+        }
+        if (f.ex.mode)
+            flag_exact(f.ex, alive && needs_exact(f.ex, nr.o.x, nr.o.y, nr.o.z, nr.d.x, nr.d.y, nr.d.z), base + out_n + rank, segment + 1);
+        out_n += (uint32_t)__popcll(mask);
+    };
+    auto load_st = [&](uint32_t idx) { return CHAIN ? load_state_chain(in, idx, segment) : load_state(in, idx, segment); };
+    auto load_hit = [&](uint32_t idx) { return f.hit4 ? make_float2(0.f, __uint_as_float(reinterpret_cast<const uint32_t *>(hits)[idx])) : qld(&hits[idx]); };
+    auto run_list = [&](uint32_t take) {
+        bool alive = false;
+        Ray nr{mk(0, 0, 0), mk(0, 0, 0)}; V3 nbeta = mk(0, 0, 0); uint32_t path_id = 0, nchain = 0;
+        if (lane < take) {
+            const uint32_t i = base + shade_list[list_n - take + lane];
+            const float4 ra = qld(&in.ray_a[i]), st = load_st(i); const float2 rb = load_ray_b(in, i, f, segment), hr = load_hit(i);
+            path_id = __float_as_uint(st.w);
+            alive = shade_path<false, CHAIN>(sc, f, objp, matp, texp, make_ray(ra, rb, f, segment), mk(st.x, st.y, st.z), __float_as_uint(st.x), path_id, hr.x, __float_as_uint(hr.y), segment, sample_rad, nr, nbeta, nchain PH_PASS);
+        }
+        list_n -= take;
+        compact(alive, nr, nbeta, nchain, path_id);
+    };
+    float4 ra_n = make_float4(0, 0, 0, 0), st_n = ra_n; float2 rb_n = make_float2(0, 0), hr_n = rb_n;
+#if FW_SHADE_PIPE
+    auto prefetch = [&](uint32_t jn) {
+        const uint32_t in_ = base + jn;
+        ra_n = qld(&in.ray_a[in_]);
+        rb_n = qld(&in.ray_b[short_rays(f, segment) ? base : in_]);
+        if (CHAIN) { const float2 v = qld(&reinterpret_cast<const float2 *>(in.state)[segment == 0 ? base : in_]); st_n = make_float4(v.x, 0.f, 0.f, v.y); }
+        else st_n = qld(&in.state[segment == 0 ? base : in_]);
+        hr_n = load_hit(in_);
+    };
+    auto fix_implicit = [&](float4 &st_, float2 &rb_, uint32_t slot) {
+        if (segment == 0) st_ = CHAIN ? make_float4(0.f, 0.f, 0.f, __uint_as_float(slot)) : make_float4(1.f, 1.f, 1.f, __uint_as_float(slot));
+        if (short_rays(f, segment)) rb_ = make_float2(0.f, 0.f);
+    };
+    if (n) {
+        prefetch(min(lane, n - 1u));
+        const uint32_t d0 = base + lane;
+        qst(&out.ray_a[d0], make_float4(0.f, 0.f, 0.f, 0.f));
+        qst(&out.ray_b[d0], make_float2(0.f, 0.f));
+        if (CHAIN) qst(&reinterpret_cast<float2 *>(out.state)[d0], make_float2(0.f, 0.f)); else qst(&out.state[d0], make_float4(0.f, 0.f, 0.f, 0.f));
+    }
+#else
+    if (lane < n) { ra_n = qld(&in.ray_a[base + lane]); rb_n = load_ray_b(in, base + lane, f, segment); st_n = load_st(base + lane); hr_n = load_hit(base + lane); }
+#endif
+    for (uint32_t c0 = 0; c0 < n; c0 += 64u) {
+        const uint32_t j = c0 + lane;
+        const uint32_t i = base + j;
+        float4 ra = ra_n, st = st_n; float2 rb = rb_n, hr = hr_n;
+#if FW_SHADE_PIPE
+        fix_implicit(st, rb, i);
+        const RngKey key_ = key_of(f, __float_as_uint(st.w));
+        prefetch(min(j + 64u, n - 1u));
+        const RngKey *pre_key = &key_;
+#else
+        if (j + 64u < n) { ra_n = qld(&in.ray_a[i + 64u]); rb_n = load_ray_b(in, i + 64u, f, segment); st_n = load_st(i + 64u); hr_n = load_hit(i + 64u); }
+        const RngKey *pre_key = nullptr;
+#endif
+        bool alive = false, later = false;
+        Ray nr{mk(0, 0, 0), mk(0, 0, 0)}; V3 nbeta = mk(0, 0, 0); uint32_t path_id = 0, nchain = 0;
+        if (j < n) {
+            PH_T0;
+            Ray r = make_ray(ra, rb, f, segment);
+            V3 beta = mk(st.x, st.y, st.z);
+            path_id = __float_as_uint(st.w);
+            const uint32_t hit_code = __float_as_uint(hr.y);
+#ifdef FW_ABL_SHADE_COPY
+            alive = hit_code != MISS && segment < 10; nr = r; nbeta = beta; nchain = __float_as_uint(st.x) + (pre_key ? pre_key->pixel & 1u : 0u);
+#else
+            if (MODE == 2 && expensive_shading(sc, objp, matp, hit_code)) later = true;
+            else alive = shade_path<MODE != 0, CHAIN>(sc, f, objp, matp, texp, r, beta, __float_as_uint(st.x), path_id, hr.x, hit_code, segment, sample_rad, nr, nbeta, nchain PH_PASS, pre_key);
+#endif
+            PH_ADD(0);
+        }
+        { PH_T0; compact(alive, nr, nbeta, nchain, path_id, c0); PH_ADD(7); }
+        if (MODE == 2) {
+            const unsigned long long lm = __ballot(later);
+            if (lm) {
+                const uint32_t lr = __builtin_amdgcn_mbcnt_hi((uint32_t)(lm >> 32), __builtin_amdgcn_mbcnt_lo((uint32_t)lm, 0u));
+                if (later) shade_list[list_n + lr] = (uint16_t)j;
+                list_n += (uint32_t)__popcll(lm);
+                if (list_n >= 64u) run_list(64u);
+            }
+        }
+    }
+    if (MODE == 2) while (list_n) run_list(min(list_n, 64u));
```

Result: faster. 44620 Mrays/s, median of 6 (+2.8%).
